# hanyujin02/trajectory_planner

Hardware: AMD Instinct MI355X
Metric: B-spline trajs/s (32 ctrl pts, 256^3 grid, 50 iters) @1 GPU; % HBM roofline (higher is better)
Workload: dtype f64

## Files before the change

trajectory_planner_amd/csrc/vigo_solver.hip:

```cpp
#include <stdlib.h>

#include <type_traits>
#include <utility>

#include "vigo_exact_div.hpp"
#include "vigo_internal.hpp"
#include "vigo_linesearch.hpp"
#include "vigo_solver_plan.hpp"

#ifndef VIGO_AXIS_TS_MARK
#define VIGO_AXIS_TS_MARK 1
#endif
#ifndef VIGO_AXIS_CONV_FILTER
#define VIGO_AXIS_CONV_FILTER 1
#endif
#ifndef VIGO_AXIS_PAIR_EVAL
#define VIGO_AXIS_PAIR_EVAL 1
#endif
#ifndef VIGO_AXIS_PAIR_UPDATE
#define VIGO_AXIS_PAIR_UPDATE 1
#endif
#ifndef VIGO_AXIS_LS_FIRST_TESTS
#define VIGO_AXIS_LS_FIRST_TESTS 0
#endif
#ifndef VIGO_AXIS_LS_FIRST_SETUP
#define VIGO_AXIS_LS_FIRST_SETUP 2
#endif

namespace vigo {
namespace {


__device__ __forceinline__ int dpp_prev_i32(int v) {
    return __builtin_amdgcn_mov_dpp(v, 0x138, 0xF, 0xF, false);
}
__device__ __forceinline__ int dpp_next_i32(int v) {
    return __builtin_amdgcn_mov_dpp(v, 0x130, 0xF, 0xF, false);
}
__device__ __forceinline__ double from_prev(double v) {
    return __hiloint2double(dpp_prev_i32(__double2hiint(v)), dpp_prev_i32(__double2loint(v)));
}
__device__ __forceinline__ double from_next(double v) {
    return __hiloint2double(dpp_next_i32(__double2hiint(v)), dpp_next_i32(__double2loint(v)));
}
__device__ __forceinline__ float from_prev(float v) {
    return __int_as_float(dpp_prev_i32(__float_as_int(v)));
}
__device__ __forceinline__ float from_next(float v) {
    return __int_as_float(dpp_next_i32(__float_as_int(v)));
}

template <typename T, int PPL>
__device__ __forceinline__ void seq_next(const T (&a)[PPL], T (&o)[PPL]) {
    const T edge = from_next(a[0]);
#pragma unroll
    for (int q = 0; q + 1 < PPL; ++q) o[q] = a[q + 1];
    o[PPL - 1] = edge;
}
template <typename T, int PPL>
__device__ __forceinline__ void seq_prev(const T (&a)[PPL], T (&o)[PPL]) {
    const T edge = from_prev(a[PPL - 1]);
#pragma unroll
    for (int q = PPL - 1; q > 0; --q) o[q] = a[q - 1];
    o[0] = edge;
}

template <int CTRL>
__device__ __forceinline__ double dpp_f64(double v) {
    const int lo = __builtin_amdgcn_mov_dpp(__double2loint(v), CTRL, 0xF, 0xF, false);
    const int hi = __builtin_amdgcn_mov_dpp(__double2hiint(v), CTRL, 0xF, 0xF, false);
    return __hiloint2double(hi, lo);
}
__device__ __forceinline__ double add_f64_again(double a, double b) {
    double r;
    asm volatile("v_add_f64 %0, %1, %2" : "=v"(r) : "v"(a), "v"(b));
    return r;
}
__device__ __forceinline__ void xor16_parts(double a, double b, double& p0, double& p1) {
    const int alo = __double2loint(a), ahi = __double2hiint(a), blo = __double2loint(b), bhi = __double2hiint(b);
    auto l = __builtin_amdgcn_permlane16_swap(alo, blo, false, false);
    auto h = __builtin_amdgcn_permlane16_swap(ahi, bhi, false, false);
    p0 = __hiloint2double(h[0], l[0]);
    p1 = __hiloint2double(h[1], l[1]);
}
__device__ __forceinline__ double xor32_sum2(double a, double b) {
    const int alo = __double2loint(a), ahi = __double2hiint(a), blo = __double2loint(b), bhi = __double2hiint(b);
    auto l = __builtin_amdgcn_permlane32_swap(alo, blo, false, false);
    auto h = __builtin_amdgcn_permlane32_swap(ahi, bhi, false, false);
    return __hiloint2double(h[0], l[0]) + __hiloint2double(h[1], l[1]);
}
__device__ __forceinline__ void xy_parts(double a, double b, double& x, double& y) {
    const int alo = __double2loint(a), ahi = __double2hiint(a), blo = __double2loint(b), bhi = __double2hiint(b);
    auto l = __builtin_amdgcn_permlane32_swap(alo, blo, false, false);
    auto h = __builtin_amdgcn_permlane32_swap(ahi, bhi, false, false);
    x = __hiloint2double(h[0], l[0]);
    y = __hiloint2double(h[1], l[1]);
}
__device__ __forceinline__ void xy_both(double v, double& x, double& y) { xy_parts(v, v, x, y); }
__device__ __forceinline__ double mul_f64_again(double a, double b) {
    double r;
    asm volatile("v_mul_f64 %0, %1, %2" : "=v"(r) : "v"(a), "v"(b));
    return r;
}
__device__ __forceinline__ double dot_xy(double a, double b) { return xor32_sum2(a * b, mul_f64_again(a, b)); }

template <int GROUP, int K>
__device__ __forceinline__ void group_sum(double (&v)[K]) {
    static_assert(GROUP == 16 || GROUP == 32 || GROUP == 64, "group is a DPP row, half a wave or a wave");
#pragma unroll
    for (int q = 0; q < K; ++q) v[q] += dpp_f64<0xB1>(v[q]);
#pragma unroll
    for (int q = 0; q < K; ++q) v[q] += dpp_f64<0x4E>(v[q]);
#pragma unroll
    for (int q = 0; q < K; ++q) v[q] += dpp_f64<0x141>(v[q]);
    if (GROUP >= 32) {
#pragma unroll
        for (int q = 0; q < K; ++q) {
            const double t = dpp_f64<0x140>(v[q]);
            const double a = v[q] + t;
            const double b = add_f64_again(v[q], t);
            double p0, p1;
            xor16_parts(a, b, p0, p1);
            if (GROUP == 64) v[q] = xor32_sum2(p0 + p1, add_f64_again(p0, p1));
            else v[q] = p0 + p1;
        }
        return;
    }
#pragma unroll
    for (int q = 0; q < K; ++q) v[q] += dpp_f64<0x140>(v[q]);
}
template <int GROUP>
__device__ __forceinline__ double group_sum1(double v) {
    double a[1] = {v};
    group_sum<GROUP, 1>(a);
    return a[0];
}

template <int K>
__device__ __forceinline__ void pair_tree32(double (&v)[K], double (&a)[K], double (&b)[K]) {
#pragma unroll
    for (int q = 0; q < K; ++q) v[q] += dpp_f64<0xB1>(v[q]);
#pragma unroll
    for (int q = 0; q < K; ++q) v[q] += dpp_f64<0x4E>(v[q]);
#pragma unroll
    for (int q = 0; q < K; ++q) v[q] += dpp_f64<0x141>(v[q]);
#pragma unroll
    for (int q = 0; q < K; ++q) {
        const double t = dpp_f64<0x140>(v[q]);
        double p0, p1;
        xor16_parts(v[q] + t, add_f64_again(v[q], t), p0, p1);
        xy_parts(p0 + p1, add_f64_again(p0, p1), a[q], b[q]);
    }
}
__device__ __forceinline__ double pack_xy(double u, double w) {
    const int ulo = __double2loint(u), uhi = __double2hiint(u), wlo = __double2loint(w), whi = __double2hiint(w);
    auto l = __builtin_amdgcn_permlane32_swap(ulo, wlo, false, false);
    auto h = __builtin_amdgcn_permlane32_swap(uhi, whi, false, false);
    return __hiloint2double(h[0], l[0]) + __hiloint2double(h[1], l[1]);
}
__device__ __forceinline__ void ys_yy_axis(double y, double s, double& ys, double& yy) {
    double v[1] = {pack_xy(y * s, y * y) + 0.0}, a[1], b[1];
    pair_tree32<1>(v, a, b);
    ys = a[0];
    yy = b[0];
}

template <int GROUP>
__device__ __forceinline__ void group_minmax(double& mn, double& mx) {
    static_assert(GROUP == 32 || GROUP == 64, "half a wave or a wave");
    auto step = [&](double omn, double omx) { mn = fmin(mn, omn); mx = fmax(mx, omx); };
    step(dpp_f64<0xB1>(mn), dpp_f64<0xB1>(mx));
    step(dpp_f64<0x4E>(mn), dpp_f64<0x4E>(mx));
    step(dpp_f64<0x141>(mn), dpp_f64<0x141>(mx));
    step(dpp_f64<0x140>(mn), dpp_f64<0x140>(mx));
    {
        double a0, a1, b0, b1;
        xor16_parts(mn, mn, a0, a1);
        xor16_parts(mx, mx, b0, b1);
        mn = fmin(a0, a1);
        mx = fmax(b0, b1);
    }
    if (GROUP == 64) {
        const int nlo = __double2loint(mn), nhi = __double2hiint(mn), xlo = __double2loint(mx), xhi = __double2hiint(mx);
        auto l = __builtin_amdgcn_permlane32_swap(nlo, nlo, false, false);
        auto h = __builtin_amdgcn_permlane32_swap(nhi, nhi, false, false);
        mn = fmin(__hiloint2double(h[0], l[0]), __hiloint2double(h[1], l[1]));
        auto l2 = __builtin_amdgcn_permlane32_swap(xlo, xlo, false, false);
        auto h2 = __builtin_amdgcn_permlane32_swap(xhi, xhi, false, false);
        mx = fmax(__hiloint2double(h2[0], l2[0]), __hiloint2double(h2[1], l2[1]));
    }
}

__device__ __forceinline__ double sum3(double a, double b, double c) { return (a + b) + c; }

__device__ __forceinline__ double fmaT(double a, double b, double c) { return __builtin_fma(a, b, c); }
__device__ __forceinline__ float fmaT(float a, float b, float c) { return __builtin_fmaf(a, b, c); }

template <bool FAST, typename T, int D = 3>
__device__ __forceinline__ double dot3(const T (&a)[3], const T (&b)[3]) {
    if (D == 2) {
        if (FAST) return fmaT((double)a[1], (double)b[1], (double)a[0] * (double)b[0]);
        return (double)a[0] * (double)b[0] + (double)a[1] * (double)b[1];
    }
    if (FAST)
        return fmaT((double)a[2], (double)b[2], fmaT((double)a[1], (double)b[1], (double)a[0] * (double)b[0]));
    return sum3((double)a[0] * (double)b[0], (double)a[1] * (double)b[1], (double)a[2] * (double)b[2]);
}
template <bool FAST, typename T, int PPL, int D = 3>
__device__ __forceinline__ double dot_lane(const T (&a)[PPL][3], const T (&b)[PPL][3]) {
    if constexpr (D == 1) {
        static_assert(!FAST && PPL == 1, "the axis-per-lane layout is reference order, one point per lane pair");
        return dot_xy((double)a[0][0], (double)b[0][0]);
    } else {
        double s = dot3<FAST, T, D>(a[0], b[0]);
#pragma unroll
        for (int q = 1; q < PPL; ++q) s += dot3<FAST, T, D>(a[q], b[q]);
        return s;
    }
}

template <bool FAST>
struct YSv {
    double v, r;
};
template <>
struct YSv<true> {
    double v;
};
__device__ __forceinline__ bool exp_in_safe_range(double a) {
    const unsigned e = ((unsigned)__double2hiint(a) >> 20) & 0x7ffu;
    return (e - 523u) < 1000u;
}
__device__ __forceinline__ YSv<true> make_ys(double ys, YSv<true>*) { return YSv<true>{1.0 / ys}; }
__device__ __forceinline__ YSv<false> make_ys(double ys, YSv<false>*) {
    return YSv<false>{ys, exp_in_safe_range(ys) ? 1.0 / ys : __builtin_nan("")};
}
template <bool MARK>
__device__ __forceinline__ double over_ys(double a, const YSv<true>& y, double&, double&) { return a * y.v; }
template <bool MARK>
__device__ __forceinline__ double over_ys(double a, const YSv<false>& y, double& amin, double& amax) {
    if (!MARK) return a / y.v;
    const double q = a * y.r;
    const double e = __builtin_fma(-q, y.v, a);
    amin = fmin(amin, fabs(a));
    amax = fmax(amax, fabs(a));
    return __builtin_fma(e, y.r, q);
}

template <bool STEADY, bool MARK>
struct TwoLoopTag {
    static constexpr bool value = STEADY;
};
template <bool FAST, bool STEADY>
constexpr bool two_loop_mark(std::integral_constant<bool, STEADY>) { return STEADY && !FAST; }
template <bool FAST, bool STEADY, bool MARK>
constexpr bool two_loop_mark(TwoLoopTag<STEADY, MARK>) { return MARK; }

template <typename T, int D = 3>
struct alignas(16) HPair {
    T s[D];
    T y[D];
};

template <typename T, int PPL>
struct LaneProblem {
    static constexpr int kGuideRegs = (PPL == 1) ? 2 : 0;
    static constexpr int kGuideDim = kGuideRegs > 0 ? kGuideRegs : 1;
    int N;
    bool level;
    int p0;
    bool has_pt[PPL];
    bool interior[PPL];
    int g_begin[PPL], g_end[PPL];
    const double* gpv;
    const uint8_t* gunk;
    T gq[kGuideDim][6];
    bool gqu[kGuideDim];
    int o_begin, o_end;
    const double* obs;
    const double* obs_tab;
    const double* obs_size;
    int o_tab, o_steps;
    double w[4];
};

__device__ __forceinline__ void hold_in_reg(double& v) { asm volatile("" : "+v"(v)); }
__device__ __forceinline__ void hold_in_reg(int& v) { asm volatile("" : "+s"(v)); }
__device__ __forceinline__ void fresh_reg(double& v) { asm volatile("" : "=v"(v)); }
__device__ __forceinline__ void fresh_reg(int& v) { asm volatile("" : "=s"(v)); }
struct HotConst {
    double dth, da, db, dc, unc_factor;
    double ts_ctrl, ts_inv_sqr;
    double g_epsilon, min_step, max_step, ftol, gtol, xtol;
    int max_iterations, max_linesearch;
    double ts_rcp, ts_lim, g_eps2;
    int conv_ok;
    __device__ __forceinline__ explicit HotConst(const DevConst& K)
        : dth(K.dth), da(K.da), db(K.db), dc(K.dc), unc_factor(K.unc_factor), ts_ctrl(K.ts_ctrl), ts_inv_sqr(K.ts_inv_sqr),
          g_epsilon(K.g_epsilon), min_step(K.min_step), max_step(K.max_step), ftol(K.ftol), gtol(K.gtol), xtol(K.xtol),
          max_iterations(K.max_iterations), max_linesearch(K.max_linesearch) {
        hold_in_reg(dth); hold_in_reg(da); hold_in_reg(db); hold_in_reg(dc); hold_in_reg(unc_factor);
        hold_in_reg(ts_ctrl); hold_in_reg(ts_inv_sqr);
        hold_in_reg(g_epsilon); hold_in_reg(min_step); hold_in_reg(max_step); hold_in_reg(ftol); hold_in_reg(gtol); hold_in_reg(xtol);
        hold_in_reg(max_iterations); hold_in_reg(max_linesearch);
        const ConstDiv cd = make_const_div(ts_ctrl);
        const ConvFilter cf = make_conv_filter(g_epsilon);
        ts_rcp = cd.r; ts_lim = cd.lim2; g_eps2 = cf.eps2;
        conv_ok = __builtin_amdgcn_readfirstlane((int)cf.ok);
        hold_in_reg(ts_rcp); hold_in_reg(ts_lim); hold_in_reg(g_eps2); hold_in_reg(conv_ok);
    }
};
template <bool HOT>
using LoopConst = std::conditional_t<HOT, HotConst, const DevConst&>;

template <typename T, class KC>
__device__ __forceinline__ bool guide_penalty(const KC& K, T dist, bool unk, T& ct, T& k, bool& scale) {
    const T dth = (T)K.dth, da = (T)K.da, db = (T)K.db, dcc = (T)K.dc;
    const T e = dth - dist;
    scale = false;
    if (e <= -dth) {
        const T ne = -e;
        ct = (ne * ne) * ne;
        k = T(3.0) * (ne * ne);
    } else if (e > T(0) && e <= dth) {
        ct = (e * e) * e;
        k = T(-3.0) * (e * e);
        scale = unk;
    } else if (e >= dth) {
        ct = (da * (e * e) + db * e) + dcc;
        k = -((T(2) * da) * e + db);
        scale = unk;
    } else {
        return false;
    }
    return true;
}
template <bool FAST, typename T>
__device__ __forceinline__ void guide_pair_term(const DevConst& K, const T (&c)[3], T px, T py, T pz, T vx,
                                                T vy, T vz, bool unk, double& cd, T (&Gd)[3]) {
    const T uf = (T)K.unc_factor;
    const T dist = FAST ? fmaT(c[2] - pz, vz, fmaT(c[1] - py, vy, (c[0] - px) * vx))
                        : ((c[0] - px) * vx + (c[1] - py) * vy) + (c[2] - pz) * vz;
    T ct, k;
    bool scale;
    if (!guide_penalty<T>(K, dist, unk, ct, k, scale)) return;
    T gx = k * vx, gy = k * vy, gz = k * vz;
    if (scale) { ct *= uf; gx *= uf; gy *= uf; gz *= uf; }
    if (!K.plan_in_z) gz = T(0.0);
    cd += (double)ct;
    Gd[0] += gx; Gd[1] += gy; Gd[2] += gz;
}
template <class KC>
__device__ __forceinline__ void guide_pair_term_axis(const KC& K, double c, double cz, double p, double pz, double v, double vz,
                                                     bool unk, double& cd, double& Gd) {
    const double uf = K.unc_factor;
    const double dist = dot_xy(c - p, v) + (cz - pz) * vz;
    double ct, k;
    bool scale;
    if (!guide_penalty<double>(K, dist, unk, ct, k, scale)) return;
    double gc = k * v;
    if (scale) { ct *= uf; gc *= uf; }
    cd += ct;
    Gd += gc;
}

template <typename T>
__device__ __forceinline__ void obstacle_term(const DevConst& K, const T (&c)[3], T opx, T opy, T ovx, T ovy, T size,
                                              double& co, T (&Go)[3]) {
    const T thr0 = (T)K.thr_dyn, oa = (T)K.oa, ob = (T)K.ob, oc = (T)K.oc;
    for (int n = 0; n <= K.pred_num; n += 2) {
        const T tn = (T)((double)n * K.ts);
        const T px = opx + tn * ovx, py = opy + tn * ovy;
        const T thr = (T(1) - (T)(n / K.pred_num) * T(0.2)) * thr0;
        const T dx = c[0] - px, dy = c[1] - py, dz = T(0.0);
        const T nrm = sqrt((dx * dx + dy * dy) + dz * dz);
        const T e = thr - (nrm - size);
        if (e > T(0)) {
            const bool cubic = e <= thr;
            const T ct = cubic ? (e * e) * e : (oa * (e * e) + ob * e) + oc;
            const T k = cubic ? T(-3.0) * (e * e) : -((T(2) * oa) * e + ob);
            co += (double)ct;
            Go[0] += k * (dx / nrm); Go[1] += k * (dy / nrm);
            if (__builtin_expect(!(nrm > T(0) && nrm < (T)INFINITY), 0)) Go[2] += k * (dz / nrm);
        }
    }
}

template <typename T>
__device__ __forceinline__ void obstacle_term_tab(const DevConst& K, const T (&c)[3], const double* tab, int steps,
                                                  T size, double& co, T (&Go)[3]) {
    const T oa = (T)K.oa, ob = (T)K.ob, oc = (T)K.oc;
    for (int s = 0; s < steps; ++s) {
        const T px = (T)tab[3 * s + 0], py = (T)tab[3 * s + 1], thr = (T)tab[3 * s + 2];
        const T dx = c[0] - px, dy = c[1] - py, dz = T(0.0);
        const T nrm = sqrt((dx * dx + dy * dy) + dz * dz);
        const T e = thr - (nrm - size);
        if (e > T(0)) {
            const bool cubic = e <= thr;
            const T ct = cubic ? (e * e) * e : (oa * (e * e) + ob * e) + oc;
            const T k = cubic ? T(-3.0) * (e * e) : -((T(2) * oa) * e + ob);
            co += (double)ct;
            Go[0] += k * (dx / nrm); Go[1] += k * (dy / nrm);
            if (__builtin_expect(!(nrm > T(0) && nrm < (T)INFINITY), 0)) Go[2] += k * (dz / nrm);
        }
    }
}

__device__ __forceinline__ bool axis_converged(const HotConst& K, double G, double X) {
    const int f = conv_filter(G, X, ConvFilter{K.g_eps2, K.conv_ok != 0});
    if (__builtin_expect(!__any(f < 0), 1)) return f != 0;
    double xnorm = sqrt(X);
    const double gnorm = sqrt(G);
    if (xnorm < 1.0) xnorm = 1.0;
    return gnorm / xnorm <= K.g_epsilon;
}

template <typename T, int PPL, bool FAST, class KC>
__device__ __forceinline__ void stencil_axis(const KC& K, const T (&C)[PPL], bool no_terms, double (&jj)[PPL],
                                             double (&vv)[PPL], double (&aa)[PPL], T (&Gs)[PPL], T (&Gf)[PPL]) {
    const T ts = (T)K.ts_ctrl, tis = (T)K.ts_inv_sqr;
    auto excess = [](T v) -> T { return v > T(1.0) ? v - T(1.0) : (v < T(-1.0) ? v + T(1.0) : T(0.0)); };
    T P1[PPL], P2[PPL], P3[PPL];
    seq_next<T, PPL>(C, P1);
    seq_next<T, PPL>(P1, P2);
    seq_next<T, PPL>(P2, P3);
    T gt0[PPL], gv[PPL], ga[PPL];
#pragma unroll
    for (int q = 0; q < PPL; ++q) {
        T J0 = FAST ? fmaT(T(3), P1[q], fmaT(T(-3), P2[q], P3[q])) - C[q]
                    : ((P3[q] - 3 * P2[q]) + 3 * P1[q]) - C[q];
        if (no_terms) J0 = T(0);
        gt0[q] = T(2.0) * J0;
        jj[q] = (double)(J0 * J0);
        constexpr bool kMark = VIGO_AXIS_TS_MARK && std::is_same_v<KC, HotConst> && std::is_same_v<T, double>;
        T evP, gq = T(0);
        if constexpr (kMark) {
            const ConstDiv cd{K.ts_ctrl, K.ts_rcp, K.ts_lim, K.ts_lim};
            T a = P1[q] - C[q];
            if (__builtin_expect(__any(!cd.usable2(a)), 0)) {
                hold_in_reg(a);
                evP = excess(a / ts);
                if (no_terms) evP = T(0);
                gq = (T(2) * evP) / ts;
            } else {
                evP = excess(cd.quotient(a));
                if (no_terms) evP = T(0);
                gq = cd.quotient(T(2) * evP);
            }
        } else {
            evP = excess((P1[q] - C[q]) / ts);
        }
        T eaP = excess((FAST ? fmaT(T(-2), P1[q], P2[q]) + C[q]
                             : (P2[q] - 2 * P1[q]) + C[q]) * tis);
        if (no_terms) { evP = T(0); eaP = T(0); }
        if constexpr (!kMark) gq = (T(2) * evP) / ts;
        gv[q] = gq * tis;
        ga[q] = (T(2) * eaP) * tis;
        vv[q] = (double)((evP * evP) * tis);
        aa[q] = (double)(eaP * eaP);
    }
    T gt1[PPL], gt2[PPL], gt3[PPL], gvM[PPL], gaM1[PPL], gaM2[PPL];
    seq_prev<T, PPL>(gt0, gt1);
    seq_prev<T, PPL>(gt1, gt2);
    seq_prev<T, PPL>(gt2, gt3);
    seq_prev<T, PPL>(gv, gvM);
    seq_prev<T, PPL>(ga, gaM1);
    seq_prev<T, PPL>(gaM1, gaM2);
#pragma unroll
    for (int q = 0; q < PPL; ++q) {
        T acc = gt3[q];
        if (FAST) {
            acc = fmaT(T(-3.0), gt2[q], acc);
            acc = fmaT(T(3.0), gt1[q], acc);
        } else {
            acc += T(-3.0) * gt2[q];
            acc += T(3.0) * gt1[q];
        }
        acc += -gt0[q];
        Gs[q] = acc;
        T fcc = gvM[q];
        fcc += -gv[q];
        fcc += gaM2[q];
        fcc += -(T(2) * gaM1[q]);
        fcc += ga[q];
        Gf[q] = fcc;
    }
}

template <typename T, int GROUP, int PPL, bool FAST, bool OBS = true, int D = 3>
__device__ __forceinline__ double eval_cost_grad(const DevConst& K, const LaneProblem<T, PPL>& Q,
                                                 const T (&c)[PPL][3], const T (&d)[PPL][3], T (&g)[PPL][3],
                                                 double (&sums)[7]) {
    using LP = LaneProblem<T, PPL>;
    const int N = Q.N;
    T Gd[PPL][3], Gs[PPL][3], Gf[PPL][3], Go[PPL][3];
    double pt_s[PPL], pt_f[PPL], pt_d[PPL], pt_o[PPL];
#pragma unroll
    for (int q = 0; q < PPL; ++q) {
        pt_s[q] = pt_f[q] = pt_d[q] = pt_o[q] = 0.0;
#pragma unroll
        for (int a = 0; a < 3; ++a) Gd[q][a] = Go[q][a] = T(0);
    }

    {
        double jj[PPL][3], vv[PPL][3], aa[PPL][3];
#pragma unroll
        for (int a = 0; a < 3; ++a) {
            if (a >= D) {
#pragma unroll
                for (int q = 0; q < PPL; ++q) { jj[q][a] = vv[q][a] = aa[q][a] = 0.0; Gs[q][a] = Gf[q][a] = T(0); }
                continue;
            }
            T C[PPL], GsA[PPL], GfA[PPL];
            double jjA[PPL], vvA[PPL], aaA[PPL];
#pragma unroll
            for (int q = 0; q < PPL; ++q) C[q] = c[q][a];
            stencil_axis<T, PPL, FAST>(K, C, a == 2 && Q.level, jjA, vvA, aaA, GsA, GfA);
#pragma unroll
            for (int q = 0; q < PPL; ++q) { jj[q][a] = jjA[q]; vv[q][a] = vvA[q]; aa[q][a] = aaA[q]; Gs[q][a] = GsA[q]; Gf[q][a] = GfA[q]; }
        }
#pragma unroll
        for (int q = 0; q < PPL; ++q) {
            const int p = Q.p0 + q;
            if (Q.has_pt[q] && p <= N - 4) pt_s[q] = sum3(jj[q][0], jj[q][1], jj[q][2]);
            double cf = 0.0;
            if (Q.has_pt[q] && p <= N - 2) cf = (vv[q][0] + vv[q][1]) + vv[q][2];
            if (Q.has_pt[q] && p <= N - 3) { cf += aa[q][0]; cf += aa[q][1]; cf += aa[q][2]; }
            pt_f[q] = cf;
        }
    }

#pragma unroll
    for (int q = 0; q < PPL; ++q) {
        if (Q.interior[q]) {
            double cd = 0.0;
            const int cnt = Q.g_end[q] - Q.g_begin[q];
#pragma unroll
            for (int j = 0; j < LP::kGuideRegs; ++j) {
                if (j < cnt)
                    guide_pair_term<FAST, T>(K, c[q], Q.gq[j][0], Q.gq[j][1], Q.gq[j][2], Q.gq[j][3], Q.gq[j][4], Q.gq[j][5],
                                       Q.gqu[j], cd, Gd[q]);
            }
            for (int j = Q.g_begin[q] + LP::kGuideRegs; j < Q.g_end[q]; ++j) {
                const double* pv = Q.gpv + 6 * (size_t)j;
                guide_pair_term<FAST, T>(K, c[q], (T)pv[0], (T)pv[1], (T)pv[2], (T)pv[3], (T)pv[4], (T)pv[5],
                                   Q.gunk ? (Q.gunk[j] != 0) : false, cd, Gd[q]);
            }
            if (K.plan_in_z) {
                const T hth = (T)K.hth, ha = (T)K.ha, hb = (T)K.hb, hc = (T)K.hc;
                const T hmin = c[q][2] - (T)K.min_h, hmax = c[q][2] - (T)K.max_h;
                if (hmin < T(0)) {
                    const T e = hth - hmin;
                    cd += (double)((ha * (e * e) + hb * e) + hc);
                    Gd[q][0] += -((T(2) * ha) * e + hb) * T(-1.0);
                } else if (hmin >= T(0) && hmax < hth) {
                    const T e = hth - hmin;
                    cd += (double)((e * e) * e);
                    Gd[q][0] += T(-3.0) * (e * e) * T(-1.0);
                }
                if (hmax > T(0)) {
                    const T e = hth + hmax;
                    cd += (double)((ha * (e * e) + hb * e) + hc);
                    Gd[q][0] += -((T(2) * ha) * e + hb) * T(1.0);
                } else if (hmax <= T(0) && hmax >= -hth) {
                    const T e = hth + hmax;
                    cd += (double)((e * e) * e);
                    Gd[q][0] += T(-3.0) * (e * e) * T(1.0);
                }
            }
            pt_d[q] = cd;
        }
    }

    if (OBS && Q.o_end > Q.o_begin) {
#pragma unroll
        for (int q = 0; q < PPL; ++q) {
            if (!Q.interior[q]) continue;
            double co = 0.0;
            for (int j = 0; j < Q.o_tab; ++j)
                obstacle_term_tab<T>(K, c[q], Q.obs_tab + 3 * j * Q.o_steps, Q.o_steps, (T)Q.obs_size[j], co, Go[q]);
            for (int j = Q.o_begin + Q.o_tab; j < Q.o_end; ++j) {
                const double* o = Q.obs + 9 * (size_t)j;
                const T hx = (T)o[6] / 2, hy = (T)o[7] / 2;
                obstacle_term<T>(K, c[q], (T)o[0], (T)o[1], (T)o[3], (T)o[4], sqrt(hx * hx + hy * hy), co, Go[q]);
            }
            pt_o[q] = co;
        }
    }

    const T w0 = (T)Q.w[0], w1 = (T)Q.w[1], w2 = (T)Q.w[2], w3 = (T)Q.w[3];
    double part[7];
#pragma unroll
    for (int q = 0; q < PPL; ++q) {
#pragma unroll
        for (int a = 0; a < 3; ++a)
            g[q][a] = (!Q.interior[q] || a >= D || (a == 2 && Q.level)) ? T(0)
                      : (FAST ? fmaT(w3, Go[q][a], fmaT(w2, Gf[q][a], fmaT(w1, Gs[q][a], w0 * Gd[q][a])))
                              : ((w0 * Gd[q][a] + w1 * Gs[q][a]) + w2 * Gf[q][a]) + w3 * Go[q][a]);
        const double v4 = dot3<FAST, T, D>(g[q], d[q]);
        const double v5 = Q.interior[q] ? dot3<FAST, T>(c[q], c[q]) : 0.0;
        const double v6 = dot3<FAST, T, D>(g[q], g[q]);
        if (q == 0) {
            part[0] = pt_d[0]; part[1] = pt_s[0]; part[2] = pt_f[0]; part[3] = pt_o[0];
            part[4] = v4; part[5] = v5; part[6] = v6;
        } else {
            part[0] += pt_d[q]; part[1] += pt_s[q]; part[2] += pt_f[q]; part[3] += pt_o[q];
            part[4] += v4; part[5] += v5; part[6] += v6;
        }
    }
    if (OBS) {
        group_sum<GROUP, 7>(part);
    } else {
        double p6[6] = {part[0], part[1], part[2], part[4], part[5], part[6]};
        group_sum<GROUP, 6>(p6);
        part[0] = p6[0]; part[1] = p6[1]; part[2] = p6[2]; part[3] = 0.0; part[4] = p6[3]; part[5] = p6[4]; part[6] = p6[5];
    }
#pragma unroll
    for (int q = 0; q < 7; ++q) sums[q] = part[q];
    return ((Q.w[0] * part[0] + Q.w[1] * part[1]) + Q.w[2] * part[2]) + Q.w[3] * part[3];
}

template <class KC>
__device__ __forceinline__ double eval_cost_grad_axis(const KC& K, const LaneProblem<double, 1>& Q, int axis,
                                                      const double (&c)[1][3], const double (&d)[1][3], double (&g)[1][3],
                                                      double (&sums)[7]) {
    using LP = LaneProblem<double, 1>;
    const int N = Q.N, p = Q.p0;
    const double C[1] = {c[0][0]};
    const double cz = c[0][2];
    double jj[1], vv[1], aa[1], Gs[1], Gf[1];
    stencil_axis<double, 1, false>(K, C, false, jj, vv, aa, Gs, Gf);
    double pt_s = 0.0, pt_f = 0.0, pt_d = 0.0;
    double pt_sf = 0.0;
    if constexpr (VIGO_AXIS_PAIR_EVAL) {
        double a0, a1;
        xy_both(aa[0], a0, a1);
        const double t = pack_xy(jj[0], vv[0]) + 0.0;
        if (Q.has_pt[0] && p <= (axis ? N - 2 : N - 4)) pt_sf = t;
        if (axis && Q.has_pt[0] && p <= N - 3) { pt_sf += a0; pt_sf += a1; pt_sf += 0.0; }
    } else {
        double j0, j1, v0, v1, a0, a1;
        xy_both(jj[0], j0, j1);
        xy_both(vv[0], v0, v1);
        xy_both(aa[0], a0, a1);
        if (Q.has_pt[0] && p <= N - 4) pt_s = sum3(j0, j1, 0.0);
        if (Q.has_pt[0] && p <= N - 2) pt_f = (v0 + v1) + 0.0;
        if (Q.has_pt[0] && p <= N - 3) { pt_f += a0; pt_f += a1; pt_f += 0.0; }
    }

    double Gd = 0.0;
    if (Q.interior[0]) {
        double cd = 0.0;
        const int cnt = Q.g_end[0] - Q.g_begin[0];
#pragma unroll
        for (int j = 0; j < LP::kGuideRegs; ++j) {
            if (j < cnt) guide_pair_term_axis(K, C[0], cz, Q.gq[j][0], Q.gq[j][2], Q.gq[j][3], Q.gq[j][5], Q.gqu[j], cd, Gd);
        }
        for (int j = Q.g_begin[0] + LP::kGuideRegs; j < Q.g_end[0]; ++j) {
            const double* pv = Q.gpv + 6 * (size_t)j;
            guide_pair_term_axis(K, C[0], cz, pv[axis], pv[2], pv[3 + axis], pv[5], Q.gunk ? (Q.gunk[j] != 0) : false, cd, Gd);
        }
        pt_d = cd;
    }

    const double w0 = Q.w[0], w1 = Q.w[1], w2 = Q.w[2], w3 = Q.w[3];
    const double Go = 0.0;
    g[0][0] = !Q.interior[0] ? 0.0 : ((w0 * Gd + w1 * Gs[0]) + w2 * Gf[0]) + w3 * Go;
    g[0][1] = g[0][2] = 0.0;
    if constexpr (VIGO_AXIS_PAIR_EVAL) {
        const double xx = dot_xy(C[0], C[0]) + cz * cz;
        double v3[3], lo[3], hi[3];
        v3[0] = axis ? (Q.interior[0] ? xx : 0.0) : pt_d;
        v3[1] = pt_sf;
        v3[2] = pack_xy(g[0][0] * d[0][0], g[0][0] * g[0][0]);
        pair_tree32<3>(v3, lo, hi);
        sums[0] = lo[0]; sums[1] = lo[1]; sums[2] = hi[1]; sums[3] = 0.0; sums[4] = lo[2]; sums[5] = hi[0]; sums[6] = hi[2];
    } else {
        double p6[6];
        p6[0] = pt_d; p6[1] = pt_s; p6[2] = pt_f;
        p6[3] = dot_xy(g[0][0], d[0][0]);
        const double xx = dot_xy(C[0], C[0]) + cz * cz;
        p6[4] = Q.interior[0] ? xx : 0.0;
        p6[5] = dot_xy(g[0][0], g[0][0]);
        group_sum<32, 6>(p6);
        sums[0] = p6[0]; sums[1] = p6[1]; sums[2] = p6[2]; sums[3] = 0.0; sums[4] = p6[3]; sums[5] = p6[4]; sums[6] = p6[5];
    }
    return ((Q.w[0] * sums[0] + Q.w[1] * sums[1]) + Q.w[2] * sums[2]) + Q.w[3] * sums[3];
}

__device__ __forceinline__ void axis_guides(LaneProblem<double, 1>& Q, int axis) {
#pragma unroll
    for (int j = 0; j < LaneProblem<double, 1>::kGuideDim; ++j) {
        Q.gq[j][0] = axis ? Q.gq[j][1] : Q.gq[j][0];
        Q.gq[j][3] = axis ? Q.gq[j][4] : Q.gq[j][3];
    }
}

template <bool MIXED> using SolveArgsOf = std::conditional_t<MIXED, MixedSolveArgs, SolveArgs>;
template <typename T, int GROUP, int PPL, bool MIXED = false>
__device__ __forceinline__ bool load_problem(const SolveArgsOf<MIXED>& A, const DevConst& K, int b, int lane_in_group,
                                             LaneProblem<T, PPL>& Q) {
    using LP = LaneProblem<T, PPL>;
    int N = A.N;
    bool valid = true;
    if constexpr (MIXED) {
        static_assert(PPL == 1, "mixed counts: one control point per lane (Ns <= 64)");
        const int n = A.n_pts[b];
        valid = n >= 7 && n <= A.N && shape_for(n).group == GROUP;
        N = valid ? n : 0;
    }
    Q.N = N;
    Q.level = false;
    Q.p0 = lane_in_group * PPL;
    Q.gpv = A.guide_pv;
    Q.gunk = A.guide_unk;
#pragma unroll
    for (int q = 0; q < PPL; ++q) {
        const int p = Q.p0 + q;
        Q.has_pt[q] = p < N;
        Q.interior[q] = (p >= 3) && (p <= N - 4);
        Q.g_begin[q] = Q.g_end[q] = 0;
        if (Q.interior[q] && A.guide_off && A.guide_pv) {
            Q.g_begin[q] = A.guide_off[(size_t)b * (MIXED ? A.N : N) + p];
            Q.g_end[q] = A.guide_off[(size_t)b * (MIXED ? A.N : N) + p + 1];
        }
    }
#pragma unroll
    for (int j = 0; j < LP::kGuideDim; ++j) {
        Q.gqu[j] = false;
#pragma unroll
        for (int q = 0; q < 6; ++q) Q.gq[j][q] = T(0);
        if (j < LP::kGuideRegs && Q.g_begin[0] + j < Q.g_end[0]) {
            const double* pv = A.guide_pv + 6 * (size_t)(Q.g_begin[0] + j);
#pragma unroll
            for (int q = 0; q < 6; ++q) Q.gq[j][q] = (T)pv[q];
            Q.gqu[j] = A.guide_unk ? (A.guide_unk[Q.g_begin[0] + j] != 0) : false;
        }
    }
    Q.obs = A.obs;
    Q.obs_tab = Q.obs_size = nullptr;
    Q.o_tab = Q.o_steps = 0;
    if (!A.obs) {
        Q.o_begin = Q.o_end = 0;
    } else if (A.obs_off) {
        Q.o_begin = A.obs_off[b];
        Q.o_end = A.obs_off[b + 1];
    } else {
        Q.o_begin = 0;
        Q.o_end = A.obs ? A.n_obs_shared : 0;
    }
    if (A.weights) {
#pragma unroll
        for (int q = 0; q < 4; ++q) Q.w[q] = A.weights[4 * (size_t)b + q];
    } else {
#pragma unroll
        for (int q = 0; q < 4; ++q) Q.w[q] = K.w[q];
    }
    return valid;
}

template <typename T, int PPL>
__device__ __forceinline__ void load_points(const SolveArgs& A, int b, const LaneProblem<T, PPL>& Q, T (&x)[PPL][3]) {
#pragma unroll
    for (int q = 0; q < PPL; ++q) {
        x[q][0] = x[q][1] = x[q][2] = T(0);
        if (Q.has_pt[q]) {
            const double* src = A.ctrl + ((size_t)b * A.N + Q.p0 + q) * 3;
            x[q][0] = (T)src[0]; x[q][1] = (T)src[1]; x[q][2] = (T)src[2];
        }
    }
}

template <typename T, int GROUP, int PPL>
__device__ __forceinline__ void set_level(const DevConst& K, LaneProblem<T, PPL>& Q, const T (&x)[PPL][3]) {
    double mn = INFINITY, mx = -INFINITY;
#pragma unroll
    for (int q = 0; q < PPL; ++q) {
        if (Q.has_pt[q]) { mn = fmin(mn, (double)x[q][2]); mx = fmax(mx, (double)x[q][2]); }
    }
    group_minmax<GROUP>(mn, mx);
    Q.level = !K.plan_in_z && !K.strict_z && (mx - mn) <= 0x1p-40 * fmax(1.0, fmax(fabs(mn), fabs(mx)));
}

template <typename T, int PPL>
__device__ __forceinline__ void store_points(const SolveArgs& A, int b, const LaneProblem<T, PPL>& Q, const T (&x)[PPL][3]) {
#pragma unroll
    for (int q = 0; q < PPL; ++q) {
        if (Q.has_pt[q]) {
            double* dst = A.ctrl + ((size_t)b * A.N + Q.p0 + q) * 3;
            dst[0] = (double)x[q][0]; dst[1] = (double)x[q][1]; dst[2] = (double)x[q][2];
        }
    }
}

__device__ __forceinline__ void store_point_axis(const SolveArgs& A, int b, const LaneProblem<double, 1>& Q, int axis, double v, double z) {
    if (!Q.has_pt[0]) return;
    double* dst = A.ctrl + ((size_t)b * A.N + Q.p0) * 3;
    dst[axis] = v;
    if (axis == 0) dst[2] = z;
}

template <typename T, int GROUP, int PPL, bool FAST, bool MIXED = false>
__global__ void __launch_bounds__(kWave) k_cost_grad(SolveArgsOf<MIXED> A, const DevConst* __restrict__ Kp) {
    const DevConst& K = *Kp;
    constexpr int TPB = kWave / GROUP;
    const int lane = threadIdx.x;
    const int b = blockIdx.x * TPB + lane / GROUP;
    if (b >= A.B) return;
    LaneProblem<T, PPL> Q;
    if (!load_problem<T, GROUP, PPL, MIXED>(A, K, b, lane % GROUP, Q)) {
        if (lane % GROUP == 0 && A.out_cost) A.out_cost[b] = __builtin_nan("");
        return;
    }
    T c[PPL][3], g[PPL][3], zero[PPL][3];
    load_points<T, PPL>(A, b, Q, c);
    set_level<T, GROUP, PPL>(K, Q, c);
#pragma unroll
    for (int q = 0; q < PPL; ++q) zero[q][0] = zero[q][1] = zero[q][2] = T(0);
    double sums[7];
    const double f = eval_cost_grad<T, GROUP, PPL, FAST>(K, Q, c, zero, g, sums);
#pragma unroll
    for (int q = 0; q < PPL; ++q) {
        if (Q.interior[q] && A.out_grad) {
            double* dst = A.out_grad + ((size_t)b * (A.N - 6) + (Q.p0 + q - 3)) * 3;
            dst[0] = (double)g[q][0]; dst[1] = (double)g[q][1]; dst[2] = (double)g[q][2];
        }
    }
    if (lane % GROUP == 0) {
        if (A.out_cost) A.out_cost[b] = f;
        if (A.out_terms) {
#pragma unroll
            for (int q = 0; q < 4; ++q) A.out_terms[4 * (size_t)b + q] = sums[q];
        }
    }
}

#ifndef VIGO_PROFILE_SECTIONS
#define VIGO_PROFILE_SECTIONS 0
#endif
#if VIGO_PROFILE_SECTIONS
#define VIGO_TICK(acc)                                                   \
    do {                                                                 \
        __builtin_amdgcn_sched_barrier(0);                               \
        const long long now_ = (long long)__builtin_readcyclecounter();  \
        __builtin_amdgcn_sched_barrier(0);                               \
        acc += (double)(now_ - tick_);                                   \
        tick_ = now_;                                                    \
    } while (0)
#else
#define VIGO_TICK(acc) do { } while (0)
#endif

template <typename T, int GROUP, int PPL, bool FAST, int WPS = 1, bool OBS = true, int D = 3, int RH = (PPL == 1 ? 1 : 0), bool MIXED = false>
__global__ void __launch_bounds__(kWave, WPS) k_optimize(SolveArgsOf<MIXED> A, const DevConst* __restrict__ Kp) {
    static_assert(!MIXED || (D == 3 && OBS && PPL == 1), "mixed counts: the general kernel, one point per lane");
    static_assert(PPL == 1 ? (RH >= 1 && RH <= 6) : RH == 0, "register-held history only with one point per lane");
    constexpr bool AXIS = D == 1;
    static_assert(!AXIS || (std::is_same<T, double>::value && GROUP == 32 && PPL == 1 && !FAST && !OBS),
                  "the axis-per-lane layout: fp64 reference order, N <= 32, no obstacles");
    const DevConst& K = *Kp;
    constexpr int TPB = AXIS ? 1 : kWave / GROUP;
    constexpr int COLS = kWave / GROUP;
    extern __shared__ __align__(16) unsigned char lds_raw[];
    const int N = A.N, NI = N - 6;
    const int ROW = COLS * NI;
    const int ROWP = ROW + 1;
    using YS = YSv<FAST>;
    constexpr int kYsSlotBytes = (TPB * (int)sizeof(YS) + 15) & ~15;
    const int slotB = ROWP * (int)sizeof(HPair<T, D>) + kYsSlotBytes;
    const int m = K.mem_size;
    const LoopConst<AXIS> KL(K);
    constexpr bool REG1 = (PPL == 1);
    const int ms = REG1 ? (m > RH + 1 ? m - (RH + 1) : 0) : m;
    HPair<T, D>* hist = reinterpret_cast<HPair<T, D>*>(lds_raw);
    double* ys_tab = reinterpret_cast<double*>(lds_raw + (size_t)ms * slotB);

    const int lane = threadIdx.x;
    const int grp = lane / GROUP;
    const int tg = AXIS ? 0 : grp;
    int b = blockIdx.x * TPB + tg;
    if (A.active_idx) {
        if (b >= *A.active_count) return;
        b = A.active_idx[b];
    } else if (b >= A.B) {
        return;
    }

    LaneProblem<T, PPL> Q;
    const bool valid_n = load_problem<T, GROUP, PPL, MIXED>(A, K, b, lane % GROUP, Q);
    T x[PPL][3];
    load_points<T, PPL>(A, b, Q, x);
    set_level<T, GROUP, PPL>(K, Q, x);
    if constexpr (AXIS) {
        if (!Q.level) return;
        x[0][0] = grp ? x[0][1] : x[0][0];
        axis_guides(Q, grp);
    } else {
        const bool wave_level = __all(Q.level);
        if (D == 2 && !wave_level) return;
        if (D == 3 && A.level_waves_elsewhere && wave_level) return;
    }
    const bool solved_elsewhere = D == 3 && A.level_waves_elsewhere == 2 && Q.level;
#if VIGO_PROFILE_SECTIONS
    long long tick_ = (long long)__builtin_readcyclecounter();
    double t_eval = 0, t_ls = 0, t_upd = 0, t_two = 0, t_tail = 0, t_pre = 0, t_trial = 0, t_cal = 0;
#endif
    HPair<T, D>* hl[PPL];
#pragma unroll
    for (int q = 0; q < PPL; ++q) {
        const int p = Q.p0 + q;
        hl[q] = Q.interior[q] ? hist + (grp * NI + (p - 3)) : hist + ROW;
    }
    for (int slot = lane; slot < ms; slot += kWave) {
        HPair<T, D> zero;
#pragma unroll
        for (int a = 0; a < D; ++a) zero.s[a] = zero.y[a] = T(0);
        *reinterpret_cast<HPair<T, D>*>(lds_raw + (size_t)slot * slotB + (size_t)ROW * sizeof(HPair<T, D>)) = zero;
    }
    __syncthreads();
    if (solved_elsewhere) return;
    if (MIXED && !valid_n) {
        if (lane % GROUP == 0 && A.out_status) A.out_status[(size_t)b * (A.status_stride ? A.status_stride : 1)] = LBERR_INVALID_N;
        return;
    }
    YS* ys_l = reinterpret_cast<YS*>(lds_raw + (size_t)ROWP * sizeof(HPair<T, D>)) + tg;
    double* al_l = ys_tab + tg;
    auto hist_at = [&](int q, int slot) -> HPair<T, D>& {
        return *reinterpret_cast<HPair<T, D>*>(reinterpret_cast<char*>(hl[q]) + (size_t)slot * slotB);
    };
    auto ys_at = [&](int slot) -> YS& { return *reinterpret_cast<YS*>(reinterpret_cast<char*>(ys_l) + (size_t)slot * slotB); };
    if (!OBS) { Q.obs = nullptr; Q.o_begin = Q.o_end = 0; }
    if (OBS && A.obs) {
        constexpr int kEnt = kObsTabEntries<GROUP>;
        double* tab = ys_tab + (size_t)m * TPB + (size_t)grp * kObsTabDoubles<GROUP>;
        const int cnt = Q.o_end - Q.o_begin;
        const int steps = K.pred_num / 2 + 1;
        int fit = kEnt / steps;
        if (fit > kObsTabObs) fit = kObsTabObs;
        Q.o_tab = cnt < fit ? cnt : fit;
        Q.o_steps = steps;
        Q.obs_tab = tab;
        Q.obs_size = tab + 3 * kEnt;
        for (int e = lane % GROUP; e < Q.o_tab * steps; e += GROUP) {
            const int j = e / steps, n = 2 * (e - j * steps);
            const double* o = A.obs + 9 * (size_t)(Q.o_begin + j);
            const T tn = (T)((double)n * K.ts);
            tab[3 * e + 0] = (double)((T)o[0] + tn * (T)o[3]);
            tab[3 * e + 1] = (double)((T)o[1] + tn * (T)o[4]);
            tab[3 * e + 2] = (double)((T(1) - (T)(n / K.pred_num) * T(0.2)) * (T)K.thr_dyn);
        }
        for (int j = lane % GROUP; j < Q.o_tab; j += GROUP) {
            const double* o = A.obs + 9 * (size_t)(Q.o_begin + j);
            const T hx = (T)o[6] / 2, hy = (T)o[7] / 2;
            tab[3 * kEnt + j] = (double)(T)sqrt(hx * hx + hy * hy);
        }
        __syncthreads();
    }

    T g[PPL][3], xp[PPL][3], gp[PPL][3], d[PPL][3];
#pragma unroll
    for (int q = 0; q < PPL; ++q)
#pragma unroll
        for (int a = 0; a < 3; ++a) g[q][a] = xp[q][a] = gp[q][a] = d[q][a] = T(0);
    constexpr int kRH = RH > 0 ? RH : 1;
    T sR[kRH][PPL][3], yR[kRH][PPL][3];
    YS ysR[kRH]{};
#pragma unroll
    for (int q = 0; q < PPL; ++q)
#pragma unroll
        for (int a = 0; a < 3; ++a)
#pragma unroll
            for (int j = 0; j < kRH; ++j) sR[j][q][a] = yR[j][q][a] = T(0);
    T dz = T(-0.0);
    double sums[7];
    int evals = 0;
    int ret = LBERR_UNKNOWN;
    int k = 0, end = 0, last = 0;
    double fx = 0.0, step = 0.0;
    bool first = true;

    for (;;) {
        int ls = 0;
        if constexpr (AXIS && (VIGO_AXIS_LS_FIRST_TESTS || VIGO_AXIS_LS_FIRST_SETUP)) {
            constexpr bool kTests = VIGO_AXIS_LS_FIRST_TESTS, kDefer = VIGO_AXIS_LS_FIRST_SETUP == 1;
            const LsParams P{KL.min_step, KL.max_step, KL.ftol, KL.gtol, KL.xtol, KL.max_linesearch};
            LsState S;
            fresh_reg(S.dginit); fresh_reg(S.finit); fresh_reg(S.dgtest); fresh_reg(S.width); fresh_reg(S.prev_width);
            fresh_reg(S.xt); fresh_reg(S.xf); fresh_reg(S.xd); fresh_reg(S.yt); fresh_reg(S.yf); fresh_reg(S.yd);
            fresh_reg(S.stmin); fresh_reg(S.stmax);
            fresh_reg(S.count); fresh_reg(S.brackt); fresh_reg(S.stage1); fresh_reg(S.uinfo);
            double step0 = step;
            auto move_x = [&]() {
                x[0][0] = xp[0][0] + step * d[0][0];
                x[0][2] = xp[0][2] + step * (Q.interior[0] ? dz : 0.0);
            };
            bool run = true;
            if (!first) {
                xp[0][0] = x[0][0]; gp[0][0] = g[0][0];
                xp[0][2] = x[0][2];
                ls = kDefer ? ls_first_begin(P, S, step, fx, sums[4]) : ls_begin(P, S, step, fx, sums[4]);
                run = ls == 0;
                if (run) {
                    if constexpr (kDefer) ls_first_setup(P, step);
                    else ls_setup(P, S, step);
                    move_x();
                }
            }
            while (run) {
                VIGO_TICK(t_pre);
                fx = eval_cost_grad_axis(KL, Q, grp, x, d, g, sums);
                VIGO_TICK(t_eval);
                ++evals;
                if (first) break;

                const double dg = sums[4];
                const double ftest1 = ls_ftest1(S, step);
                ++S.count;
                if ((kTests || kDefer) && S.count == 1) {
                    if constexpr (kTests) {
                        const int code = ls_first_exit_code(P, S, step, fx, dg, ftest1);
                        if (__any(code != 0)) { ls = code; break; }
                    }
                    if constexpr (kDefer) {
                        hold_in_reg(step0);
                        ls_first_reject(P, S, step0);
                        hold_in_reg(S.xt); hold_in_reg(S.xf); hold_in_reg(S.xd); hold_in_reg(S.yt); hold_in_reg(S.yf); hold_in_reg(S.yd);
                        hold_in_reg(S.width); hold_in_reg(S.prev_width); hold_in_reg(S.stmin); hold_in_reg(S.stmax);
                        hold_in_reg(S.brackt); hold_in_reg(S.stage1); hold_in_reg(S.uinfo);
                    }
                }
                if (!kTests || S.count != 1) {
                    const int code = ls_exit_code(P, S, step, fx, dg, ftest1);
                    if (code != 0) { ls = code; break; }
                }
                VIGO_TICK(t_ls);
                ls_update(P, S, step, fx, dg, ftest1);
                VIGO_TICK(t_trial);
                ls_setup(P, S, step);
                move_x();
            }
        } else {
            int count = 0, brackt = 0, stage1 = 1, uinfo = 0;
            double dginit = 0.0, finit = 0.0, dgtest = 0.0, width = 0.0, prev_width = 0.0;
            double xt = 0., xf = 0., xd = 0., yt = 0., yf = 0., yd = 0.;
            const double stpmin = KL.min_step, stpmax = KL.max_step;
            bool run = true;
            if (!first) {
#pragma unroll
                for (int q = 0; q < PPL; ++q)
#pragma unroll
                    for (int a = 0; a < D; ++a) { xp[q][a] = x[q][a]; gp[q][a] = g[q][a]; }
                if constexpr (AXIS) xp[0][2] = x[0][2];
                dginit = sums[4];
                if (step <= 0.) { ls = LBERR_INVALIDPARAMETERS; run = false; }
                else if (0 < dginit) { ls = LBERR_INCREASEGRADIENT; run = false; }
                finit = fx;
                dgtest = KL.ftol * dginit;
                width = stpmax - stpmin;
                prev_width = 2.0 * width;
                xt = yt = 0.;
                xf = yf = finit;
                xd = yd = dginit;
            }
            while (run) {
                double stmin = 0., stmax = 0.;
                if (!first) {
                    if (brackt) {
                        stmin = xt <= yt ? xt : yt;
                        stmax = xt >= yt ? xt : yt;
                    } else {
                        stmin = xt;
                        stmax = step + 4.0 * (step - xt);
                    }
                    if (step < stpmin) step = stpmin;
                    if (stpmax < step) step = stpmax;
                    if ((brackt && ((step <= stmin || stmax <= step) || KL.max_linesearch <= count + 1 || uinfo != 0)) ||
                        (brackt && (stmax - stmin <= KL.xtol * stmax))) {
                        step = xt;
                    }
#pragma unroll
                    for (int q = 0; q < PPL; ++q)
#pragma unroll
                        for (int a = 0; a < D; ++a)
                            x[q][a] = FAST ? fmaT((T)step, d[q][a], xp[q][a]) : xp[q][a] + (T)step * d[q][a];
                    if constexpr (AXIS) x[0][2] = xp[0][2] + (T)step * (Q.interior[0] ? dz : T(0));
                }

                VIGO_TICK(t_pre);
                if constexpr (AXIS) fx = eval_cost_grad_axis(KL, Q, grp, x, d, g, sums);
                else fx = eval_cost_grad<T, GROUP, PPL, FAST, OBS, D>(KL, Q, x, d, g, sums);
                VIGO_TICK(t_eval);
                ++evals;
                if (first) break;

                const double dg = sums[4];
                const double ftest1 = finit + step * dgtest;
                ++count;

                {
                    int code = 0;
                    if (fx <= ftest1 && fabs(dg) <= KL.gtol * (-dginit)) code = count;
                    if (KL.max_linesearch <= count) code = LBERR_MAXIMUMLINESEARCH;
                    if (brackt && (stmax - stmin) <= KL.xtol * stmax) code = LBERR_WIDTHTOOSMALL;
                    if (step == stpmin && (ftest1 < fx || dgtest <= dg)) code = LBERR_MINIMUMSTEP;
                    if (step == stpmax && fx <= ftest1 && dg <= dgtest) code = LBERR_MAXIMUMSTEP;
                    if (brackt && ((step <= stmin || stmax <= step) || uinfo != 0)) code = LBERR_ROUNDING_ERROR;
                    if (code != 0) { ls = code; break; }
                }

                const double cmin = KL.ftol <= KL.gtol ? KL.ftol : KL.gtol;
                if (stage1 && fx <= ftest1 && cmin * dginit <= dg) stage1 = 0;

                const bool mod = stage1 && ftest1 < fx && fx <= xf;
                double axf = mod ? xf - xt * dgtest : xf, axd = mod ? xd - dgtest : xd;
                double ayf = mod ? yf - yt * dgtest : yf, ayd = mod ? yd - dgtest : yd;
                const double atf = mod ? fx - step * dgtest : fx, atd = mod ? dg - dgtest : dg;
                VIGO_TICK(t_ls);
                uinfo = trial_interval(xt, axf, axd, yt, ayf, ayd, step, atf, atd, stmin, stmax, brackt);
                VIGO_TICK(t_trial);
                xf = mod ? axf + xt * dgtest : axf;
                yf = mod ? ayf + yt * dgtest : ayf;
                xd = mod ? axd + dgtest : axd;
                yd = mod ? ayd + dgtest : ayd;

                if (brackt) {
                    if (0.66 * prev_width <= fabs(yt - xt)) step = xt + 0.5 * (yt - xt);
                    prev_width = width;
                    width = fabs(yt - xt);
                }
            }
        }

        VIGO_TICK(t_ls);
        double xnorm = sqrt(sums[5]), gnorm = sqrt(sums[6]);
        if (first) {
            first = false;
#pragma unroll
            for (int q = 0; q < PPL; ++q)
#pragma unroll
                for (int a = 0; a < D; ++a) d[q][a] = -g[q][a];
            if constexpr (AXIS && VIGO_AXIS_CONV_FILTER) {
                if (axis_converged(KL, sums[6], sums[5])) { ret = LB_ALREADY_MINIMIZED; break; }
            } else {
                if (xnorm < 1.0) xnorm = 1.0;
                if (gnorm / xnorm <= KL.g_epsilon) { ret = LB_ALREADY_MINIMIZED; break; }
            }
            step = 1.0 / sqrt(sums[6]);
            sums[4] = -sums[6];
            k = 1;
            end = 0;
            continue;
        }

        if (ls < 0) {
            if constexpr (AXIS) store_point_axis(A, b, Q, grp, Q.interior[0] ? x[0][0] : xp[0][0], Q.interior[0] ? x[0][2] : xp[0][2]);
            else store_points<T, PPL>(A, b, Q, x);
#pragma unroll
            for (int q = 0; q < PPL; ++q)
#pragma unroll
                for (int a = 0; a < D; ++a) { x[q][a] = xp[q][a]; g[q][a] = gp[q][a]; }
            if constexpr (AXIS) x[0][2] = xp[0][2];
            ret = ls;
            break;
        }

        if constexpr (AXIS && VIGO_AXIS_CONV_FILTER) {
            if (axis_converged(KL, sums[6], sums[5])) { ret = LB_CONVERGENCE; break; }
        } else {
            if (xnorm < 1.0) xnorm = 1.0;
            if (gnorm / xnorm <= KL.g_epsilon) { ret = LB_CONVERGENCE; break; }
        }
        if (KL.max_iterations != 0 && KL.max_iterations < k + 1) { ret = LBERR_MAXIMUMITERATION; break; }

        T sv[PPL][3], yv[PPL][3];
#pragma unroll
        for (int q = 0; q < PPL; ++q) {
#pragma unroll
            for (int a = 0; a < D; ++a) { sv[q][a] = x[q][a] - xp[q][a]; yv[q][a] = g[q][a] - gp[q][a]; }
            if (!REG1 && Q.interior[q]) {
                HPair<T, D> hp;
#pragma unroll
                for (int a = 0; a < D; ++a) { hp.s[a] = sv[q][a]; hp.y[a] = yv[q][a]; }
                hist_at(q, end) = hp;
            }
        }
        double ysyy[2];
        if constexpr (AXIS && VIGO_AXIS_PAIR_UPDATE) {
            ys_yy_axis(yv[0][0], sv[0][0], ysyy[0], ysyy[1]);
        } else {
            ysyy[0] = dot_lane<FAST, T, PPL, D>(yv, sv);
            ysyy[1] = dot_lane<FAST, T, PPL, D>(yv, yv);
            if (D <= 2) ysyy[0] += 0.0;
            group_sum<GROUP, 2>(ysyy);
        }
        const double ys = ysyy[0], yy = ysyy[1];
        const YS ys_div = make_ys(ys, static_cast<YS*>(nullptr));
        if (!REG1) ys_at(end) = ys_div;
        const bool haveR = REG1 && k >= RH + 1;

        const int bound = (m <= k) ? m : k;
        const int newest = REG1 ? last : end;
        if (!REG1) end = (end + 1 == m) ? 0 : end + 1;
        ++k;
#pragma unroll
        for (int q = 0; q < PPL; ++q)
#pragma unroll
            for (int a = 0; a < D; ++a) d[q][a] = -g[q][a];

        constexpr int kWin = 2;
        T Ps[kWin][PPL][3], Py[kWin][PPL][3];
        YS Pys[kWin];
        auto fetch = [&](int age, T (&s_)[PPL][3], T (&y_)[PPL][3], YS& ys_) {
            if (REG1 && age == 0) {
#pragma unroll
                for (int q = 0; q < PPL; ++q)
#pragma unroll
                    for (int a = 0; a < D; ++a) { s_[q][a] = sv[q][a]; y_[q][a] = yv[q][a]; }
                ys_ = ys_div;
                return;
            }
            if (REG1 && age >= 1 && age <= RH) {
                const int j = (age - 1 < kRH && age >= 1) ? age - 1 : 0;
#pragma unroll
                for (int q = 0; q < PPL; ++q)
#pragma unroll
                    for (int a = 0; a < D; ++a) { s_[q][a] = sR[j][q][a]; y_[q][a] = yR[j][q][a]; }
                ys_ = ysR[j];
                return;
            }
            int slot = REG1 ? newest - (age - (RH + 1)) : newest - age;
            if (slot < 0) slot += ms;
#pragma unroll
            for (int q = 0; q < PPL; ++q) {
                const HPair<T, D> h = hist_at(q, slot);
#pragma unroll
                for (int a = 0; a < D; ++a) { s_[q][a] = h.s[a]; y_[q][a] = h.y[a]; }
            }
            ys_ = ys_at(slot);
        };
        auto two_loop = [&](auto steady_tag) -> bool {
            constexpr bool STEADY = decltype(steady_tag)::value;
            constexpr bool MARK = two_loop_mark<FAST>(decltype(steady_tag){});
            double amin = 1.0, amax = 1.0;
            const int bnd = STEADY ? kMaxMem : __builtin_amdgcn_readfirstlane(bound);
            constexpr bool REGAL = STEADY || AXIS;
            double al_reg[REGAL ? kMaxMem : 1];
            constexpr int kRing = kMaxMem - (RH + 1);
            constexpr int kFirstRing = RH + 1;
            const int stepB = slotB;
            const int lastU = STEADY ? __builtin_amdgcn_readfirstlane(last) : 0;
            int curB = lastU * stepB;
            auto ring_fetch = [&](T (&s_)[PPL][3], T (&y_)[PPL][3], YS& ys_) {
#pragma unroll
                for (int q = 0; q < PPL; ++q) {
                    const HPair<T, D> h = *reinterpret_cast<const HPair<T, D>*>(reinterpret_cast<const char*>(hl[q]) + curB);
#pragma unroll
                    for (int a = 0; a < D; ++a) { s_[q][a] = h.s[a]; y_[q][a] = h.y[a]; }
                }
                ys_ = *reinterpret_cast<const YS*>(reinterpret_cast<const char*>(ys_l) + curB);
            };
            auto ring_older = [&]() {
                curB -= stepB;
                if (curB < 0) curB += kRing * stepB;
            };
            auto ring_newer = [&]() {
                curB += stepB;
                if (curB >= kRing * stepB) curB -= kRing * stepB;
            };
            auto ring_fetch_age = [&](int age, bool newer_next, T (&s_)[PPL][3], T (&y_)[PPL][3], YS& ys_) {
                ring_fetch(s_, y_, ys_);
                if (newer_next) ring_newer(); else ring_older();
            };
#pragma unroll
            for (int q = 0; q < PPL; ++q)
#pragma unroll
                for (int a = 0; a < D; ++a) { Ps[0][q][a] = sv[q][a]; Py[0][q][a] = yv[q][a]; }
            Pys[0] = ys_div;
#pragma unroll
            for (int age = 1; age < kWin; ++age)
                if (age < bnd) {
                    if (STEADY && age >= kFirstRing) ring_fetch_age(age, false, Ps[age], Py[age], Pys[age]);
                    else fetch(age, Ps[age], Py[age], Pys[age]);
                }
#pragma unroll
            for (int age = 0; age < kMaxMem; ++age) {
                if (age < bnd) {
                    const int w = age % kWin;
                    double al = group_sum1<GROUP>(dot_lane<FAST, T, PPL, D>(Ps[w], d));
                    al = over_ys<MARK>(al, Pys[w], amin, amax);
                    if (REGAL) al_reg[REGAL ? age : 0] = al;
                    else al_l[age * TPB] = al;
                    {
                        const T na = (T)(-al);
#pragma unroll
                        for (int q = 0; q < PPL; ++q)
#pragma unroll
                            for (int a = 0; a < D; ++a) d[q][a] = FAST ? fmaT(na, Py[w][q][a], d[q][a]) : d[q][a] + na * Py[w][q][a];
                    }
                    if (age + kWin < kMaxMem && age + kWin < bnd) {
                        if (STEADY && age + kWin >= kFirstRing) ring_fetch_age(age + kWin, false, Ps[w], Py[w], Pys[w]);
                        else fetch(age + kWin, Ps[w], Py[w], Pys[w]);
                    }
                }
            }
            if (STEADY) {
#pragma unroll
                for (int i = 0; i < kWin + 1; ++i) ring_newer();
                asm volatile("" ::: "memory");
            }
            {
                const T sc = (T)(ys / yy);
#pragma unroll
                for (int q = 0; q < PPL; ++q)
#pragma unroll
                    for (int a = 0; a < D; ++a) d[q][a] *= sc;
            }
#pragma unroll
            for (int age = kMaxMem - 1; age >= 0; --age) {
                if (age < bnd) {
                    const int w = age % kWin;
                    double beta = group_sum1<GROUP>(dot_lane<FAST, T, PPL, D>(Py[w], d));
                    beta = over_ys<MARK>(beta, Pys[w], amin, amax);
                    const double cod = (REGAL ? al_reg[REGAL ? age : 0] : al_l[age * TPB]) - beta;
                    {
                        const T co = (T)cod;
#pragma unroll
                        for (int q = 0; q < PPL; ++q)
#pragma unroll
                            for (int a = 0; a < D; ++a) d[q][a] = FAST ? fmaT(co, Ps[w][q][a], d[q][a]) : d[q][a] + co * Ps[w][q][a];
                    }
                    if (age - kWin >= 0) {
                        if (STEADY && age - kWin >= kFirstRing) ring_fetch_age(age - kWin, true, Ps[w], Py[w], Pys[w]);
                        else fetch(age - kWin, Ps[w], Py[w], Pys[w]);
                    }
                }
            }
            if (!MARK) return false;
            bool bad = !(amin >= 0x1p-500) || !(amax <= 0x1p500);
#pragma unroll
            for (int q = 0; q < PPL; ++q)
#pragma unroll
                for (int a = 0; a < D; ++a) bad |= !(d[q][a] == d[q][a]);
            return bad;
        };
        VIGO_TICK(t_upd);
        if constexpr (AXIS) {
            bool bad;
            if (bound == kMaxMem && !__any(last != __builtin_amdgcn_readfirstlane(last))) bad = two_loop(TwoLoopTag<true, true>{});
            else bad = two_loop(TwoLoopTag<false, true>{});
            if (__any(bad)) {
                asm volatile("" ::: "memory");
                d[0][0] = -g[0][0];
                two_loop(TwoLoopTag<false, false>{});
            }
        } else if (PPL == 1 && bound == kMaxMem && !__any(last != __builtin_amdgcn_readfirstlane(last))) {
            if (__any(two_loop(std::true_type{}))) {
                asm volatile("" ::: "memory");
#pragma unroll
                for (int q = 0; q < PPL; ++q)
#pragma unroll
                    for (int a = 0; a < D; ++a) d[q][a] = -g[q][a];
                two_loop(std::false_type{});
            }
        } else {
            two_loop(std::false_type{});
        }
        if constexpr (AXIS)
            dz = __hiloint2double(__builtin_amdgcn_readfirstlane(__double2hiint(d[0][0])),
                                  __builtin_amdgcn_readfirstlane(__double2loint(d[0][0])));
#pragma unroll
        for (int q = 0; q < PPL; ++q)
#pragma unroll
            for (int a = 0; a < D; ++a) d[q][a] = Q.interior[q] ? d[q][a] : T(0);
        VIGO_TICK(t_two);
        if (REG1) {
            if (haveR && ms > 0) {
#pragma unroll
                for (int q = 0; q < PPL; ++q) {
                    if (Q.interior[q]) {
                        HPair<T, D> hp;
#pragma unroll
                        for (int a = 0; a < D; ++a) { hp.s[a] = sR[kRH - 1][q][a]; hp.y[a] = yR[kRH - 1][q][a]; }
                        hist_at(q, end) = hp;
                    }
                }
                ys_at(end) = ysR[kRH - 1];
                last = end;
                end = (end + 1 == ms) ? 0 : end + 1;
            }
#pragma unroll
            for (int j = kRH - 1; j > 0; --j) {
#pragma unroll
                for (int q = 0; q < PPL; ++q)
#pragma unroll
                    for (int a = 0; a < D; ++a) { sR[j][q][a] = sR[j - 1][q][a]; yR[j][q][a] = yR[j - 1][q][a]; }
                ysR[j] = ysR[j - 1];
            }
#pragma unroll
            for (int q = 0; q < PPL; ++q)
#pragma unroll
                for (int a = 0; a < D; ++a) { sR[0][q][a] = sv[q][a]; yR[0][q][a] = yv[q][a]; }
            ysR[0] = ys_div;
        }
        sums[4] = group_sum1<GROUP>(dot_lane<FAST, T, PPL, D>(g, d));
        step = 1.0;
        VIGO_TICK(t_tail);
        VIGO_TICK(t_cal);
    }

    if (ret >= 0 || ret == LBERR_MAXIMUMITERATION) {
        if constexpr (AXIS) store_point_axis(A, b, Q, grp, x[0][0], x[0][2]);
        else store_points<T, PPL>(A, b, Q, x);
    }
#pragma unroll
    for (int q = 0; q < PPL; ++q) {
        if (Q.interior[q] && A.out_x) {
            double* dst = A.out_x + ((size_t)b * NI + (Q.p0 + q - 3)) * 3;
            if constexpr (AXIS) {
                dst[grp] = (double)x[q][0];
                if (grp == 0) dst[2] = (double)x[q][2];
            } else {
                dst[0] = (double)x[q][0]; dst[1] = (double)x[q][1]; dst[2] = (double)x[q][2];
            }
        }
    }
#if VIGO_PROFILE_SECTIONS
    if (lane % GROUP == 0 && A.out_x) {
        double* o = A.out_x + (size_t)b * NI * 3;
        o[0] = t_eval; o[1] = t_ls; o[2] = t_upd; o[3] = t_two; o[4] = t_tail; o[5] = (double)k; o[6] = (double)evals;
        o[7] = t_pre; o[8] = t_trial; o[9] = t_cal;
    }
#endif
    if (lane % (kWave / TPB) == 0) {
        if (A.out_status) A.out_status[(size_t)b * (A.status_stride ? A.status_stride : 1)] = ret;
        if (A.out_fx) A.out_fx[b] = fx;
        if (A.out_iters) A.out_iters[b] = k;
        if (A.out_evals) A.out_evals[b] = evals;
    }
}

}

#ifndef VIGO_SOLVER_PART
#define VIGO_SOLVER_PART 0
#endif

using SolveKernel = void (*)(SolveArgs, const DevConst*);
using MixedSolveKernel = void (*)(MixedSolveArgs, const DevConst*);

#if VIGO_SOLVER_PART == 0
DevConst make_dev_const(const vigo_params_t& P) {
    DevConst K{};
    K.dth = P.dthresh;
    K.da = 3.0 * P.dthresh;
    K.db = -3.0 * pow(P.dthresh, 2);
    K.dc = pow(P.dthresh, 3);
    K.unc_factor = P.uncertain_factor;
    K.hth = 0.2;
    K.ha = 3.0 * K.hth;
    K.hb = -3 * pow(K.hth, 2);
    K.hc = pow(K.hth, 3);
    K.min_h = P.min_height;
    K.max_h = P.max_height;
    K.ts_ctrl = P.ts_ctrl;
    K.ts_inv_sqr = 1 / pow(P.ts_ctrl, 2);
    K.ts = P.ts;
    K.thr_dyn = P.dist_thresh_dynamic;
    K.oa = 3.0 * P.dist_thresh_dynamic;
    K.ob = -3 * pow(P.dist_thresh_dynamic, 2);
    K.oc = pow(P.dist_thresh_dynamic, 3);
    K.pred_num = (int)(P.pred_horizon / P.ts);
    K.plan_in_z = P.plan_in_z;
    K.strict_z = P.strict_z != 0;
    K.w[0] = P.w_distance; K.w[1] = P.w_smoothness; K.w[2] = P.w_feasibility; K.w[3] = P.w_dynamic;
    K.mem_size = P.mem_size;
    K.max_iterations = P.max_iterations;
    K.max_linesearch = P.max_linesearch;
    K.g_epsilon = P.g_epsilon;
    K.min_step = P.min_step;
    K.max_step = P.max_step;
    K.ftol = P.f_dec_coeff;
    K.gtol = P.s_curv_coeff;
    K.xtol = P.xtol;
    return K;
}

int launch_cost_grad(hipStream_t s, const SolveArgs& a, const DevConst&, const DevConst* kd, int precision) {
    if (a.B <= 0) return hipSuccess;
    static constexpr SolveKernel kernels[3][4] = {
        {&k_cost_grad<float, 32, 1, false>, &k_cost_grad<float, 64, 1, false>, &k_cost_grad<float, 64, 2, false>, &k_cost_grad<float, 64, 4, false>},
        {&k_cost_grad<double, 32, 1, true>, &k_cost_grad<double, 64, 1, true>, &k_cost_grad<double, 64, 2, true>, &k_cost_grad<double, 64, 4, true>},
        {&k_cost_grad<double, 32, 1, false>, &k_cost_grad<double, 64, 1, false>, &k_cost_grad<double, 64, 2, false>, &k_cost_grad<double, 64, 4, false>}};
    const Shape sh = shape_for(a.N);
    const int tpb = kWave / sh.group;
    const SolveKernel kernel = kernels[precision == VIGO_PREC_F32 ? 0 : (precision == VIGO_PREC_F64_FAST ? 1 : 2)]
                                      [sh.ppl == 1 ? sh.group / 64 : sh.ppl / 2 + 1];
    hipLaunchKernelGGL(kernel, dim3((a.B + tpb - 1) / tpb), dim3(kWave), 0, s, a, kd);
    return (int)hipGetLastError();
}
#endif


template <int I>
static constexpr SolveKernel optimize_kernel_of() {
    constexpr OptimizeKey k = kOptimizeKeys[I];
    if constexpr (VIGO_SOLVER_PART <= 1 && k.obs == (VIGO_SOLVER_PART == 1)) {
        using T = std::conditional_t<k.precision == VIGO_PREC_F32, float, double>;
        constexpr bool FAST = k.precision == VIGO_PREC_F64_FAST;
        static_assert(sizeof(T) == elem_bytes_of(k.precision) && sizeof(HPair<T, k.d>) == hpair_bytes(sizeof(T), k.d) &&
                          sizeof(YSv<FAST>) == ysv_bytes(FAST), "optimize_lds_bytes computes these sizes by arithmetic");
        return &k_optimize<T, k.group, k.ppl, FAST, k.wps, k.obs, k.d, k.rh>;
    }
    return nullptr;
}
template <class Rows> struct OptimizeKernelTable;
template <int... I> struct OptimizeKernelTable<std::integer_sequence<int, I...>> { static constexpr SolveKernel row[] = {optimize_kernel_of<I>()...}; };
static SolveKernel optimize_kernel(int key) { return OptimizeKernelTable<std::make_integer_sequence<int, kOptimizeKeyCount>>::row[key]; }

#if VIGO_SOLVER_PART == 2
template <int I>
static constexpr MixedSolveKernel optimize_mixed_kernel_of() {
    constexpr OptimizeKey k = kOptimizeMixedKeys[I];
    using T = std::conditional_t<k.precision == VIGO_PREC_F32, float, double>;
    constexpr bool FAST = k.precision == VIGO_PREC_F64_FAST;
    static_assert(sizeof(T) == elem_bytes_of(k.precision) && sizeof(HPair<T, k.d>) == hpair_bytes(sizeof(T), k.d) &&
                      sizeof(YSv<FAST>) == ysv_bytes(FAST), "optimize_lds_bytes computes these sizes by arithmetic");
    return &k_optimize<T, k.group, k.ppl, FAST, k.wps, k.obs, k.d, k.rh, true>;
}
template <class Rows> struct OptimizeMixedKernelTable;
template <int... I> struct OptimizeMixedKernelTable<std::integer_sequence<int, I...>> { static constexpr MixedSolveKernel row[] = {optimize_mixed_kernel_of<I>()...}; };
MixedSolveKernel optimize_mixed_kernel(int key) { return OptimizeMixedKernelTable<std::make_integer_sequence<int, kOptimizeMixedKeyCount>>::row[key]; }
MixedSolveKernel cost_grad_mixed_kernel(int precision, int group) {
    static constexpr MixedSolveKernel kernels[3][2] = {
        {&k_cost_grad<float, 32, 1, false, true>, &k_cost_grad<float, 64, 1, false, true>},
        {&k_cost_grad<double, 32, 1, true, true>, &k_cost_grad<double, 64, 1, true, true>},
        {&k_cost_grad<double, 32, 1, false, true>, &k_cost_grad<double, 64, 1, false, true>}};
    return kernels[precision == VIGO_PREC_F32 ? 0 : (precision == VIGO_PREC_F64_FAST ? 1 : 2)][group / 64];
}
#elif VIGO_SOLVER_PART == 1
SolveKernel optimize_kernel_with_obstacles(int key) { return optimize_kernel(key); }
#else
SolveKernel optimize_kernel_with_obstacles(int key);
MixedSolveKernel optimize_mixed_kernel(int key);
MixedSolveKernel cost_grad_mixed_kernel(int precision, int group);
#ifndef VIGO_EXP_AXIS_SWITCH
#define VIGO_EXP_AXIS_SWITCH 0
#endif
static inline bool axis_dispatch_on() {
#if VIGO_EXP_AXIS_SWITCH
    const char* e = getenv("VIGO_EXP_AXIS");
    return !(e && e[0] == '0');
#else
    return true;
#endif
}

int launch_optimize(hipStream_t s, const SolveArgs& a_in, const DevConst& k, const DevConst* kd, int precision, LaunchState& L) {
    static_assert(kOptimizeKeyCount <= 8 * (int)sizeof(L.lds_attr_set), "one bit per k_optimize instantiation");
    if (a_in.B <= 0) return hipSuccess;
    const OptimizePlan plan = plan_optimize(a_in.N, a_in.B, precision, a_in.obs != nullptr, k.plan_in_z != 0, k.strict_z != 0,
                                            k.mem_size, L.simd_count, axis_dispatch_on());
    if (plan.count < 0) return (int)hipErrorInvalidValue;
    SolveArgs a = a_in;
    for (int i = 0; i < plan.count; ++i) {
        const PlannedLaunch& p = plan.launch[i];
        const SolveKernel kernel = kOptimizeKeys[p.key].obs ? optimize_kernel_with_obstacles(p.key) : optimize_kernel(p.key);
        const uint64_t bit = 1ull << p.key;
        if (p.lds > kLdsStaticLimit && !(L.lds_attr_set & bit)) {
            hipError_t e = hipFuncSetAttribute(reinterpret_cast<const void*>(kernel), hipFuncAttributeMaxDynamicSharedMemorySize, (int)kLdsPerWorkgroup);
            if (e != hipSuccess) return (int)e;
            L.lds_attr_set |= bit;
        }
        a.level_waves_elsewhere = p.level_waves_elsewhere;
        hipLaunchKernelGGL(kernel, dim3(p.grid), dim3(kWave), p.lds, s, a, kd);
        if (hipError_t e = hipGetLastError(); e != hipSuccess) return (int)e;
    }
    return (int)hipSuccess;
}

int launch_cost_grad_mixed(hipStream_t s, const MixedSolveArgs& a, const DevConst* kd, int precision) {
    if (a.B <= 0) return hipSuccess;
    const Shape sh = shape_for(a.N);
    if (sh.ppl != 1 || !a.n_pts) return (int)hipErrorInvalidValue;
    const int tpb = kWave / sh.group;
    hipLaunchKernelGGL(cost_grad_mixed_kernel(precision, sh.group), dim3((a.B + tpb - 1) / tpb), dim3(kWave), 0, s, a, kd);
    return (int)hipGetLastError();
}
int launch_optimize_mixed(hipStream_t s, const MixedSolveArgs& a_in, const DevConst& k, const DevConst* kd, int precision, LaunchState& L) {
    if (a_in.B <= 0) return hipSuccess;
    const OptimizePlan plan = plan_optimize_mixed(a_in.N, a_in.B, precision, a_in.obs != nullptr, k.mem_size, L.simd_count);
    if (plan.count != 1 || !a_in.n_pts) return (int)hipErrorInvalidValue;
    const PlannedLaunch& p = plan.launch[0];
    MixedSolveArgs a = a_in;
    a.level_waves_elsewhere = p.level_waves_elsewhere;
    hipLaunchKernelGGL(optimize_mixed_kernel(p.key), dim3(p.grid), dim3(kWave), p.lds, s, a, kd);
    return (int)hipGetLastError();
}
#endif

}
```

trajectory_planner_amd/csrc/vigo_solver_plan.hpp:

```cpp
#pragma once
#include <stddef.h>

#include "../../include/vigo.h"

namespace vigo {

constexpr int kWave = 64;
constexpr size_t kLdsPerWorkgroup = 160 * 1024;
constexpr size_t kLdsStaticLimit = 64 * 1024;
constexpr int kMaxMem = VIGO_MAX_MEM_SIZE;
constexpr int kObsTabObs = 16;
template <int GROUP> constexpr int kObsTabEntries = GROUP == 32 ? 88 : 33;
template <int GROUP> constexpr int kObsTabDoubles = 3 * kObsTabEntries<GROUP> + kObsTabObs;
constexpr int kLevelRH = 4, kLevelRH64 = 5;
struct Shape { int group, ppl; };
constexpr Shape shape_for(int N) { return N <= 32 ? Shape{32, 1} : Shape{64, N <= 64 ? 1 : (N <= 128 ? 2 : 4)}; }
constexpr int default_rh(int ppl) { return ppl == 1 ? 1 : 0; }
constexpr size_t elem_bytes_of(int precision) { return precision == VIGO_PREC_F32 ? 4 : 8; }
constexpr size_t hpair_bytes(size_t elem_bytes, int D) { return (2 * D * elem_bytes + 15) & ~(size_t)15; }
constexpr size_t ysv_bytes(bool fast) { return fast ? 8 : 16; }

constexpr size_t optimize_lds_bytes(size_t elem_bytes, int group, bool fast, int D, int N, int m, int ppl, bool with_obstacles, int rh) {
    const int TPB = D == 1 ? 1 : kWave / group;
    const int COLS = kWave / group;
    const int ms = ppl == 1 ? (m > rh + 1 ? m - (rh + 1) : 0) : m;
    const size_t slot = ((size_t)COLS * (N - 6) + 1) * hpair_bytes(elem_bytes, D) + (((size_t)TPB * ysv_bytes(fast) + 15) & ~(size_t)15);
    size_t h = (size_t)ms * slot;
    h += (size_t)m * TPB * sizeof(double);
    if (with_obstacles) h += (size_t)TPB * (group == 32 ? kObsTabDoubles<32> : kObsTabDoubles<64>) * sizeof(double);
    return h;
}

constexpr size_t optimize_lds_requirement(int N, int mem_size, int precision) {
    const Shape sh = shape_for(N);
    return optimize_lds_bytes(elem_bytes_of(precision), sh.group, precision == VIGO_PREC_F64_FAST, 3, N, mem_size, sh.ppl, true, default_rh(sh.ppl));
}

struct OptimizeKey { int precision, group, ppl, wps; bool obs; int d, rh; };
constexpr int kF32 = VIGO_PREC_F32, kFast = VIGO_PREC_F64_FAST, kF64 = VIGO_PREC_F64;
constexpr OptimizeKey kOptimizeKeys[] = {
    {kF32, 32, 1, 2, false, 2, 1}, {kF32, 32, 1, 1, false, 2, 1}, {kF32, 32, 1, 2, false, 3, 1}, {kF32, 32, 1, 1, false, 3, 1},
    {kF32, 64, 1, 2, false, 2, 1}, {kF32, 64, 1, 1, false, 2, 1}, {kF32, 64, 1, 2, false, 3, 1}, {kF32, 64, 1, 1, false, 3, 1},
    {kF32, 64, 2, 1, false, 3, 0}, {kF32, 64, 4, 1, false, 3, 0},
    {kFast, 32, 1, 2, false, 2, kLevelRH}, {kFast, 32, 1, 2, false, 2, 1}, {kFast, 32, 1, 1, false, 2, 1}, {kFast, 32, 1, 2, false, 3, 1}, {kFast, 32, 1, 1, false, 3, 1},
    {kFast, 64, 1, 2, false, 2, kLevelRH64}, {kFast, 64, 1, 2, false, 2, 1}, {kFast, 64, 1, 1, false, 2, 1}, {kFast, 64, 1, 2, false, 3, 1}, {kFast, 64, 1, 1, false, 3, 1},
    {kFast, 64, 2, 1, false, 3, 0}, {kFast, 64, 4, 1, false, 3, 0},
    {kF64, 32, 1, 1, false, 1, 1},
    {kF64, 32, 1, 2, false, 2, kLevelRH}, {kF64, 32, 1, 2, false, 2, 1}, {kF64, 32, 1, 1, false, 2, 1}, {kF64, 32, 1, 2, false, 3, 1}, {kF64, 32, 1, 1, false, 3, 1},
    {kF64, 64, 1, 2, false, 2, kLevelRH64}, {kF64, 64, 1, 2, false, 2, 1}, {kF64, 64, 1, 1, false, 2, 1}, {kF64, 64, 1, 2, false, 3, 1}, {kF64, 64, 1, 1, false, 3, 1},
    {kF64, 64, 2, 1, false, 3, 0}, {kF64, 64, 4, 1, false, 3, 0},
    {kF32, 32, 1, 2, true, 3, 1}, {kF32, 32, 1, 1, true, 3, 1}, {kF32, 64, 1, 2, true, 3, 1}, {kF32, 64, 1, 1, true, 3, 1},
    {kF32, 64, 2, 1, true, 3, 0}, {kF32, 64, 4, 1, true, 3, 0},
    {kFast, 32, 1, 2, true, 3, 1}, {kFast, 32, 1, 1, true, 3, 1}, {kFast, 64, 1, 2, true, 3, 1}, {kFast, 64, 1, 1, true, 3, 1},
    {kFast, 64, 2, 1, true, 3, 0}, {kFast, 64, 4, 1, true, 3, 0},
    {kF64, 32, 1, 2, true, 3, 1}, {kF64, 32, 1, 1, true, 3, 1}, {kF64, 64, 1, 2, true, 3, 1}, {kF64, 64, 1, 1, true, 3, 1},
    {kF64, 64, 2, 1, true, 3, 0}, {kF64, 64, 4, 1, true, 3, 0},
};
constexpr int kOptimizeKeyCount = sizeof(kOptimizeKeys) / sizeof(kOptimizeKeys[0]);
constexpr int optimize_key_index(const OptimizeKey& k) {
    for (int i = 0; i < kOptimizeKeyCount; ++i) {
        const OptimizeKey& c = kOptimizeKeys[i];
        if (c.precision == k.precision && c.group == k.group && c.ppl == k.ppl && c.wps == k.wps && c.obs == k.obs && c.d == k.d && c.rh == k.rh) return i;
    }
    return -1;
}

struct PlannedLaunch { int key, grid; size_t lds; int level_waves_elsewhere; };
struct OptimizePlan { int count; PlannedLaunch launch[2]; };

inline OptimizePlan plan_optimize(int N, int B, int precision, bool has_obstacle_list, bool plan_in_z, bool strict_z, int mem_size, int simd_count, bool allow_axis) {
    const Shape sh = shape_for(N);
    const size_t eb = elem_bytes_of(precision);
    const bool fast = precision == VIGO_PREC_F64_FAST, f64 = precision == VIGO_PREC_F64;
    const bool obs = has_obstacle_list || (fast && N > 32 && N <= 64 && simd_count > 0 && B > simd_count && (plan_in_z || strict_z));
    const int grid = (B + kWave / sh.group - 1) / (kWave / sh.group);
    const bool crowded = grid > (simd_count > 0 ? simd_count : (1 << 30));
    auto lds_of = [&](int D, bool table, int rh) { return optimize_lds_bytes(eb, sh.group, fast, D, N, mem_size, sh.ppl, table, rh); };
    auto wps_for = [&](size_t lds) { return sh.ppl == 1 && crowded && lds <= kLdsPerWorkgroup / 8 ? 2 : 1; };
    OptimizePlan p{};
    auto add = [&](int wps, int D, int rh, int g, size_t lds, int lwe) {
        const int key = optimize_key_index(OptimizeKey{precision, sh.group, sh.ppl, wps, obs, D, rh});
        if (key < 0 || p.count < 0) p.count = -1;
        else p.launch[p.count++] = PlannedLaunch{key, g, lds, lwe};
    };
    const size_t lds = lds_of(3, has_obstacle_list, default_rh(sh.ppl));
    if (lds > kLdsPerWorkgroup) return OptimizePlan{-1, {}};
    int lwe = 0;
    if (sh.ppl == 1 && !obs && !plan_in_z && !strict_z) {
        lwe = 1;
        const int rh = sh.group == 32 ? kLevelRH : kLevelRH64;
        const size_t lds2 = lds_of(2, false, 1), lds3 = lds_of(2, false, rh);
        if (f64 && sh.group == 32 && simd_count > 0 && B <= simd_count && allow_axis) {
            add(1, 1, 1, B, lds_of(1, false, 1), lwe);
            lwe = 2;
        } else if (precision != VIGO_PREC_F32 && crowded && lds2 > kLdsPerWorkgroup / 8 && kLdsPerWorkgroup / lds3 > kLdsPerWorkgroup / lds2) {
            add(2, 2, rh, grid, lds3, lwe);
        } else {
            add(wps_for(lds2), 2, 1, grid, lds2, lwe);
        }
    }
    add(wps_for(lds), 3, default_rh(sh.ppl), grid, lds, lwe);
    return p;
}

constexpr int kMixedMaxStride = 64;
constexpr OptimizeKey kOptimizeMixedKeys[] = {
    {kF32, 32, 1, 2, true, 3, 1}, {kF32, 32, 1, 1, true, 3, 1}, {kF32, 64, 1, 2, true, 3, 1}, {kF32, 64, 1, 1, true, 3, 1},
    {kFast, 32, 1, 2, true, 3, 1}, {kFast, 32, 1, 1, true, 3, 1}, {kFast, 64, 1, 2, true, 3, 1}, {kFast, 64, 1, 1, true, 3, 1},
    {kF64, 32, 1, 2, true, 3, 1}, {kF64, 32, 1, 1, true, 3, 1}, {kF64, 64, 1, 2, true, 3, 1}, {kF64, 64, 1, 1, true, 3, 1},
};
constexpr int kOptimizeMixedKeyCount = sizeof(kOptimizeMixedKeys) / sizeof(kOptimizeMixedKeys[0]);
constexpr int optimize_mixed_key_index(int precision, int group, int wps) {
    for (int i = 0; i < kOptimizeMixedKeyCount; ++i) {
        const OptimizeKey& c = kOptimizeMixedKeys[i];
        if (c.precision == precision && c.group == group && c.wps == wps) return i;
    }
    return -1;
}
constexpr bool mixed_count_ok(int n, int Ns) { return n >= 7 && n <= Ns && Ns <= kMixedMaxStride && shape_for(n).group == shape_for(Ns).group; }

inline OptimizePlan plan_optimize_mixed(int Ns, int B, int precision, bool , int mem_size, int simd_count) {
    if (Ns < 7 || Ns > kMixedMaxStride) return OptimizePlan{-1, {}};
    const Shape sh = shape_for(Ns);
    const int grid = (B + kWave / sh.group - 1) / (kWave / sh.group);
    const bool crowded = grid > (simd_count > 0 ? simd_count : (1 << 30));
    const size_t lds = optimize_lds_bytes(elem_bytes_of(precision), sh.group, precision == VIGO_PREC_F64_FAST, 3, Ns, mem_size, 1, true, 1);
    const int key = optimize_mixed_key_index(precision, sh.group, crowded && lds <= kLdsPerWorkgroup / 8 ? 2 : 1);
    if (key < 0 || lds > kLdsStaticLimit) return OptimizePlan{-1, {}};
    return OptimizePlan{1, {PlannedLaunch{key, grid, lds, 0}, {}}};
}

}
```

Measured before the change: 3.897 million.

## Fuse axis-per-lane and general optimize kernels into one launch per trajectory

Moves the optimize kernel body into a shared include and adds a fused kernel. Each block loads its problem once, then branches to the axis-per-lane solver for level trajectories or to a noinline solo general solver otherwise. This replaces the previous two-launch plan (axis kernel, then a general kernel that skipped already-solved waves) and removes one launch plus the redundant problem load. The cost is a larger register footprint from combining both paths, and LDS sized for the larger of the two.

New measurement: 3.956 million, median of 6. 1.5% higher.

```diff
diff --git a/trajectory_planner_amd/csrc/vigo_solver.hip b/trajectory_planner_amd/csrc/vigo_solver.hip
--- a/trajectory_planner_amd/csrc/vigo_solver.hip
+++ b/trajectory_planner_amd/csrc/vigo_solver.hip
@@ -853,589 +853,87 @@
 
 template <typename T, int GROUP, int PPL, bool FAST, int WPS = 1, bool OBS = true, int D = 3, int RH = (PPL == 1 ? 1 : 0), bool MIXED = false>
 __global__ void __launch_bounds__(kWave, WPS) k_optimize(SolveArgsOf<MIXED> A, const DevConst* __restrict__ Kp) {
-    static_assert(!MIXED || (D == 3 && OBS && PPL == 1), "mixed counts: the general kernel, one point per lane");
-    static_assert(PPL == 1 ? (RH >= 1 && RH <= 6) : RH == 0, "register-held history only with one point per lane");
-    constexpr bool AXIS = D == 1;
-    static_assert(!AXIS || (std::is_same<T, double>::value && GROUP == 32 && PPL == 1 && !FAST && !OBS),
-                  "the axis-per-lane layout: fp64 reference order, N <= 32, no obstacles");
+    constexpr bool SOLO = false;
+#define VIGO_OPTIMIZE_ENTRY 1
+#include "vigo_solver_optimize.inc"
+#undef VIGO_OPTIMIZE_ENTRY
+}
+
+template <typename T, int GROUP, int PPL, bool FAST, bool OBS, int D, bool SOLO>
+__device__ __forceinline__ void optimize_loaded(const SolveArgs& A, const DevConst& K, const LoopConst<D == 1>& KL, const int b,
+                                                LaneProblem<T, PPL>& Q, T (&x)[PPL][3]) {
+    constexpr int RH = 1;
+    constexpr bool MIXED = false;
+    const bool valid_n = true;
+#define VIGO_OPTIMIZE_ENTRY 0
+#include "vigo_solver_optimize.inc"
+#undef VIGO_OPTIMIZE_ENTRY
+}
+
+#ifndef VIGO_FUSED_JOIN
+#define VIGO_FUSED_JOIN 0
+#endif
+#if VIGO_FUSED_JOIN == 2
+struct FusedKernArgs { SolveArgs A; const DevConst* Kp; };
+template <class P>
+__device__ __forceinline__ const P& uniform_constant(const void* p) {
+    const unsigned long long u = (unsigned long long)p;
+    const unsigned long long lo = (unsigned)__builtin_amdgcn_readfirstlane((int)(unsigned)u);
+    const unsigned long long hi = (unsigned)__builtin_amdgcn_readfirstlane((int)(unsigned)(u >> 32));
+    typedef const P __attribute__((address_space(4))) * CP;
+    return *(const P*)(CP)((hi << 32) | lo);
+}
+__device__ __noinline__ void optimize_solo(const void* kernargs, const int b_in, const LaneProblem<double, 1>& Q_in, const double (&x_in)[1][3]) {
+    const FusedKernArgs& F = uniform_constant<FusedKernArgs>(kernargs);
+    const DevConst& K = uniform_constant<DevConst>(F.Kp);
+    const int b = __builtin_amdgcn_readfirstlane(b_in);
+    LaneProblem<double, 1> Q = Q_in;
+    double x[1][3] = {{x_in[0][0], x_in[0][1], x_in[0][2]}};
+    optimize_loaded<double, 32, 1, false, false, 3, true>(F.A, K, K, b, Q, x);
+}
+#elif VIGO_FUSED_JOIN == 0
+__device__ __noinline__ void optimize_solo(const SolveArgs& A, const DevConst* Kp, const int b, LaneProblem<double, 1>& Q, double (&x)[1][3]) {
+    optimize_loaded<double, 32, 1, false, false, 3, true>(A, *Kp, *Kp, b, Q, x);
+}
+#endif
+template <int WPS>
+__global__ void __launch_bounds__(kWave, WPS) k_optimize_fused(SolveArgs A, const DevConst* __restrict__ Kp) {
     const DevConst& K = *Kp;
-    constexpr int TPB = AXIS ? 1 : kWave / GROUP;
-    constexpr int COLS = kWave / GROUP;
-    extern __shared__ __align__(16) unsigned char lds_raw[];
-    const int N = A.N, NI = N - 6;
-    const int ROW = COLS * NI;
-    const int ROWP = ROW + 1;
-    using YS = YSv<FAST>;
-    constexpr int kYsSlotBytes = (TPB * (int)sizeof(YS) + 15) & ~15;
-    const int slotB = ROWP * (int)sizeof(HPair<T, D>) + kYsSlotBytes;
-    const int m = K.mem_size;
-    const LoopConst<AXIS> KL(K);
-    constexpr bool REG1 = (PPL == 1);
-    const int ms = REG1 ? (m > RH + 1 ? m - (RH + 1) : 0) : m;
-    HPair<T, D>* hist = reinterpret_cast<HPair<T, D>*>(lds_raw);
-    double* ys_tab = reinterpret_cast<double*>(lds_raw + (size_t)ms * slotB);
-
+    const HotConst KL(K);
     const int lane = threadIdx.x;
-    const int grp = lane / GROUP;
-    const int tg = AXIS ? 0 : grp;
-    int b = blockIdx.x * TPB + tg;
+    const int grp = lane / 32;
+    int b = blockIdx.x;
     if (A.active_idx) {
         if (b >= *A.active_count) return;
         b = A.active_idx[b];
     } else if (b >= A.B) {
         return;
     }
-
-    LaneProblem<T, PPL> Q;
-    const bool valid_n = load_problem<T, GROUP, PPL, MIXED>(A, K, b, lane % GROUP, Q);
-    T x[PPL][3];
-    load_points<T, PPL>(A, b, Q, x);
-    set_level<T, GROUP, PPL>(K, Q, x);
-    if constexpr (AXIS) {
-        if (!Q.level) return;
+    LaneProblem<double, 1> Q;
+    load_problem<double, 32, 1>(A, K, b, lane % 32, Q);
+    double x[1][3];
+    load_points<double, 1>(A, b, Q, x);
+    set_level<double, 32, 1>(K, Q, x);
+    if (__builtin_amdgcn_readfirstlane((int)Q.level)) {
         x[0][0] = grp ? x[0][1] : x[0][0];
         axis_guides(Q, grp);
+        optimize_loaded<double, 32, 1, false, false, 1, false>(A, K, KL, b, Q, x);
     } else {
-        const bool wave_level = __all(Q.level);
-        if (D == 2 && !wave_level) return;
-        if (D == 3 && A.level_waves_elsewhere && wave_level) return;
-    }
-    const bool solved_elsewhere = D == 3 && A.level_waves_elsewhere == 2 && Q.level;
-#if VIGO_PROFILE_SECTIONS
-    long long tick_ = (long long)__builtin_readcyclecounter();
-    double t_eval = 0, t_ls = 0, t_upd = 0, t_two = 0, t_tail = 0, t_pre = 0, t_trial = 0, t_cal = 0;
-#endif
-    HPair<T, D>* hl[PPL];
-#pragma unroll
-    for (int q = 0; q < PPL; ++q) {
-        const int p = Q.p0 + q;
-        hl[q] = Q.interior[q] ? hist + (grp * NI + (p - 3)) : hist + ROW;
-    }
-    for (int slot = lane; slot < ms; slot += kWave) {
-        HPair<T, D> zero;
-#pragma unroll
-        for (int a = 0; a < D; ++a) zero.s[a] = zero.y[a] = T(0);
-        *reinterpret_cast<HPair<T, D>*>(lds_raw + (size_t)slot * slotB + (size_t)ROW * sizeof(HPair<T, D>)) = zero;
-    }
-    __syncthreads();
-    if (solved_elsewhere) return;
-    if (MIXED && !valid_n) {
-        if (lane % GROUP == 0 && A.out_status) A.out_status[(size_t)b * (A.status_stride ? A.status_stride : 1)] = LBERR_INVALID_N;
-        return;
-    }
-    YS* ys_l = reinterpret_cast<YS*>(lds_raw + (size_t)ROWP * sizeof(HPair<T, D>)) + tg;
-    double* al_l = ys_tab + tg;
-    auto hist_at = [&](int q, int slot) -> HPair<T, D>& {
-        return *reinterpret_cast<HPair<T, D>*>(reinterpret_cast<char*>(hl[q]) + (size_t)slot * slotB);
-    };
-    auto ys_at = [&](int slot) -> YS& { return *reinterpret_cast<YS*>(reinterpret_cast<char*>(ys_l) + (size_t)slot * slotB); };
-    if (!OBS) { Q.obs = nullptr; Q.o_begin = Q.o_end = 0; }
-    if (OBS && A.obs) {
-        constexpr int kEnt = kObsTabEntries<GROUP>;
-        double* tab = ys_tab + (size_t)m * TPB + (size_t)grp * kObsTabDoubles<GROUP>;
-        const int cnt = Q.o_end - Q.o_begin;
-        const int steps = K.pred_num / 2 + 1;
-        int fit = kEnt / steps;
-        if (fit > kObsTabObs) fit = kObsTabObs;
-        Q.o_tab = cnt < fit ? cnt : fit;
-        Q.o_steps = steps;
-        Q.obs_tab = tab;
-        Q.obs_size = tab + 3 * kEnt;
-        for (int e = lane % GROUP; e < Q.o_tab * steps; e += GROUP) {
-            const int j = e / steps, n = 2 * (e - j * steps);
-            const double* o = A.obs + 9 * (size_t)(Q.o_begin + j);
-            const T tn = (T)((double)n * K.ts);
-            tab[3 * e + 0] = (double)((T)o[0] + tn * (T)o[3]);
-            tab[3 * e + 1] = (double)((T)o[1] + tn * (T)o[4]);
-            tab[3 * e + 2] = (double)((T(1) - (T)(n / K.pred_num) * T(0.2)) * (T)K.thr_dyn);
-        }
-        for (int j = lane % GROUP; j < Q.o_tab; j += GROUP) {
-            const double* o = A.obs + 9 * (size_t)(Q.o_begin + j);
-            const T hx = (T)o[6] / 2, hy = (T)o[7] / 2;
-            tab[3 * kEnt + j] = (double)(T)sqrt(hx * hx + hy * hy);
-        }
-        __syncthreads();
-    }
-
-    T g[PPL][3], xp[PPL][3], gp[PPL][3], d[PPL][3];
-#pragma unroll
-    for (int q = 0; q < PPL; ++q)
-#pragma unroll
-        for (int a = 0; a < 3; ++a) g[q][a] = xp[q][a] = gp[q][a] = d[q][a] = T(0);
-    constexpr int kRH = RH > 0 ? RH : 1;
-    T sR[kRH][PPL][3], yR[kRH][PPL][3];
-    YS ysR[kRH]{};
-#pragma unroll
-    for (int q = 0; q < PPL; ++q)
-#pragma unroll
-        for (int a = 0; a < 3; ++a)
-#pragma unroll
-            for (int j = 0; j < kRH; ++j) sR[j][q][a] = yR[j][q][a] = T(0);
-    T dz = T(-0.0);
-    double sums[7];
-    int evals = 0;
-    int ret = LBERR_UNKNOWN;
-    int k = 0, end = 0, last = 0;
-    double fx = 0.0, step = 0.0;
-    bool first = true;
-
-    for (;;) {
-        int ls = 0;
-        if constexpr (AXIS && (VIGO_AXIS_LS_FIRST_TESTS || VIGO_AXIS_LS_FIRST_SETUP)) {
-            constexpr bool kTests = VIGO_AXIS_LS_FIRST_TESTS, kDefer = VIGO_AXIS_LS_FIRST_SETUP == 1;
-            const LsParams P{KL.min_step, KL.max_step, KL.ftol, KL.gtol, KL.xtol, KL.max_linesearch};
-            LsState S;
-            fresh_reg(S.dginit); fresh_reg(S.finit); fresh_reg(S.dgtest); fresh_reg(S.width); fresh_reg(S.prev_width);
-            fresh_reg(S.xt); fresh_reg(S.xf); fresh_reg(S.xd); fresh_reg(S.yt); fresh_reg(S.yf); fresh_reg(S.yd);
-            fresh_reg(S.stmin); fresh_reg(S.stmax);
-            fresh_reg(S.count); fresh_reg(S.brackt); fresh_reg(S.stage1); fresh_reg(S.uinfo);
-            double step0 = step;
-            auto move_x = [&]() {
-                x[0][0] = xp[0][0] + step * d[0][0];
-                x[0][2] = xp[0][2] + step * (Q.interior[0] ? dz : 0.0);
-            };
-            bool run = true;
-            if (!first) {
-                xp[0][0] = x[0][0]; gp[0][0] = g[0][0];
-                xp[0][2] = x[0][2];
-                ls = kDefer ? ls_first_begin(P, S, step, fx, sums[4]) : ls_begin(P, S, step, fx, sums[4]);
-                run = ls == 0;
-                if (run) {
-                    if constexpr (kDefer) ls_first_setup(P, step);
-                    else ls_setup(P, S, step);
-                    move_x();
-                }
-            }
-            while (run) {
-                VIGO_TICK(t_pre);
-                fx = eval_cost_grad_axis(KL, Q, grp, x, d, g, sums);
-                VIGO_TICK(t_eval);
-                ++evals;
-                if (first) break;
-
-                const double dg = sums[4];
-                const double ftest1 = ls_ftest1(S, step);
-                ++S.count;
-                if ((kTests || kDefer) && S.count == 1) {
-                    if constexpr (kTests) {
-                        const int code = ls_first_exit_code(P, S, step, fx, dg, ftest1);
-                        if (__any(code != 0)) { ls = code; break; }
-                    }
-                    if constexpr (kDefer) {
-                        hold_in_reg(step0);
-                        ls_first_reject(P, S, step0);
-                        hold_in_reg(S.xt); hold_in_reg(S.xf); hold_in_reg(S.xd); hold_in_reg(S.yt); hold_in_reg(S.yf); hold_in_reg(S.yd);
-                        hold_in_reg(S.width); hold_in_reg(S.prev_width); hold_in_reg(S.stmin); hold_in_reg(S.stmax);
-                        hold_in_reg(S.brackt); hold_in_reg(S.stage1); hold_in_reg(S.uinfo);
-                    }
-                }
-                if (!kTests || S.count != 1) {
-                    const int code = ls_exit_code(P, S, step, fx, dg, ftest1);
-                    if (code != 0) { ls = code; break; }
-                }
-                VIGO_TICK(t_ls);
-                ls_update(P, S, step, fx, dg, ftest1);
-                VIGO_TICK(t_trial);
-                ls_setup(P, S, step);
-                move_x();
-            }
-        } else {
-            int count = 0, brackt = 0, stage1 = 1, uinfo = 0;
-            double dginit = 0.0, finit = 0.0, dgtest = 0.0, width = 0.0, prev_width = 0.0;
-            double xt = 0., xf = 0., xd = 0., yt = 0., yf = 0., yd = 0.;
-            const double stpmin = KL.min_step, stpmax = KL.max_step;
-            bool run = true;
-            if (!first) {
-#pragma unroll
-                for (int q = 0; q < PPL; ++q)
-#pragma unroll
-                    for (int a = 0; a < D; ++a) { xp[q][a] = x[q][a]; gp[q][a] = g[q][a]; }
-                if constexpr (AXIS) xp[0][2] = x[0][2];
-                dginit = sums[4];
-                if (step <= 0.) { ls = LBERR_INVALIDPARAMETERS; run = false; }
-                else if (0 < dginit) { ls = LBERR_INCREASEGRADIENT; run = false; }
-                finit = fx;
-                dgtest = KL.ftol * dginit;
-                width = stpmax - stpmin;
-                prev_width = 2.0 * width;
-                xt = yt = 0.;
-                xf = yf = finit;
-                xd = yd = dginit;
-            }
-            while (run) {
-                double stmin = 0., stmax = 0.;
-                if (!first) {
-                    if (brackt) {
-                        stmin = xt <= yt ? xt : yt;
-                        stmax = xt >= yt ? xt : yt;
-                    } else {
-                        stmin = xt;
-                        stmax = step + 4.0 * (step - xt);
-                    }
-                    if (step < stpmin) step = stpmin;
-                    if (stpmax < step) step = stpmax;
-                    if ((brackt && ((step <= stmin || stmax <= step) || KL.max_linesearch <= count + 1 || uinfo != 0)) ||
-                        (brackt && (stmax - stmin <= KL.xtol * stmax))) {
-                        step = xt;
-                    }
-#pragma unroll
-                    for (int q = 0; q < PPL; ++q)
-#pragma unroll
-                        for (int a = 0; a < D; ++a)
-                            x[q][a] = FAST ? fmaT((T)step, d[q][a], xp[q][a]) : xp[q][a] + (T)step * d[q][a];
-                    if constexpr (AXIS) x[0][2] = xp[0][2] + (T)step * (Q.interior[0] ? dz : T(0));
-                }
-
-                VIGO_TICK(t_pre);
-                if constexpr (AXIS) fx = eval_cost_grad_axis(KL, Q, grp, x, d, g, sums);
-                else fx = eval_cost_grad<T, GROUP, PPL, FAST, OBS, D>(KL, Q, x, d, g, sums);
-                VIGO_TICK(t_eval);
-                ++evals;
-                if (first) break;
-
-                const double dg = sums[4];
-                const double ftest1 = finit + step * dgtest;
-                ++count;
-
-                {
-                    int code = 0;
-                    if (fx <= ftest1 && fabs(dg) <= KL.gtol * (-dginit)) code = count;
-                    if (KL.max_linesearch <= count) code = LBERR_MAXIMUMLINESEARCH;
-                    if (brackt && (stmax - stmin) <= KL.xtol * stmax) code = LBERR_WIDTHTOOSMALL;
-                    if (step == stpmin && (ftest1 < fx || dgtest <= dg)) code = LBERR_MINIMUMSTEP;
-                    if (step == stpmax && fx <= ftest1 && dg <= dgtest) code = LBERR_MAXIMUMSTEP;
-                    if (brackt && ((step <= stmin || stmax <= step) || uinfo != 0)) code = LBERR_ROUNDING_ERROR;
-                    if (code != 0) { ls = code; break; }
-                }
-
-                const double cmin = KL.ftol <= KL.gtol ? KL.ftol : KL.gtol;
-                if (stage1 && fx <= ftest1 && cmin * dginit <= dg) stage1 = 0;
-
-                const bool mod = stage1 && ftest1 < fx && fx <= xf;
-                double axf = mod ? xf - xt * dgtest : xf, axd = mod ? xd - dgtest : xd;
-                double ayf = mod ? yf - yt * dgtest : yf, ayd = mod ? yd - dgtest : yd;
-                const double atf = mod ? fx - step * dgtest : fx, atd = mod ? dg - dgtest : dg;
-                VIGO_TICK(t_ls);
-                uinfo = trial_interval(xt, axf, axd, yt, ayf, ayd, step, atf, atd, stmin, stmax, brackt);
-                VIGO_TICK(t_trial);
-                xf = mod ? axf + xt * dgtest : axf;
-                yf = mod ? ayf + yt * dgtest : ayf;
-                xd = mod ? axd + dgtest : axd;
-                yd = mod ? ayd + dgtest : ayd;
-
-                if (brackt) {
-                    if (0.66 * prev_width <= fabs(yt - xt)) step = xt + 0.5 * (yt - xt);
-                    prev_width = width;
-                    width = fabs(yt - xt);
-                }
-            }
-        }
-
-        VIGO_TICK(t_ls);
-        double xnorm = sqrt(sums[5]), gnorm = sqrt(sums[6]);
-        if (first) {
-            first = false;
-#pragma unroll
-            for (int q = 0; q < PPL; ++q)
-#pragma unroll
-                for (int a = 0; a < D; ++a) d[q][a] = -g[q][a];
-            if constexpr (AXIS && VIGO_AXIS_CONV_FILTER) {
-                if (axis_converged(KL, sums[6], sums[5])) { ret = LB_ALREADY_MINIMIZED; break; }
-            } else {
-                if (xnorm < 1.0) xnorm = 1.0;
-                if (gnorm / xnorm <= KL.g_epsilon) { ret = LB_ALREADY_MINIMIZED; break; }
-            }
-            step = 1.0 / sqrt(sums[6]);
-            sums[4] = -sums[6];
-            k = 1;
-            end = 0;
-            continue;
-        }
-
-        if (ls < 0) {
-            if constexpr (AXIS) store_point_axis(A, b, Q, grp, Q.interior[0] ? x[0][0] : xp[0][0], Q.interior[0] ? x[0][2] : xp[0][2]);
-            else store_points<T, PPL>(A, b, Q, x);
-#pragma unroll
-            for (int q = 0; q < PPL; ++q)
-#pragma unroll
-                for (int a = 0; a < D; ++a) { x[q][a] = xp[q][a]; g[q][a] = gp[q][a]; }
-            if constexpr (AXIS) x[0][2] = xp[0][2];
-            ret = ls;
-            break;
-        }
-
-        if constexpr (AXIS && VIGO_AXIS_CONV_FILTER) {
-            if (axis_converged(KL, sums[6], sums[5])) { ret = LB_CONVERGENCE; break; }
-        } else {
-            if (xnorm < 1.0) xnorm = 1.0;
-            if (gnorm / xnorm <= KL.g_epsilon) { ret = LB_CONVERGENCE; break; }
-        }
-        if (KL.max_iterations != 0 && KL.max_iterations < k + 1) { ret = LBERR_MAXIMUMITERATION; break; }
-
-        T sv[PPL][3], yv[PPL][3];
-#pragma unroll
-        for (int q = 0; q < PPL; ++q) {
-#pragma unroll
-            for (int a = 0; a < D; ++a) { sv[q][a] = x[q][a] - xp[q][a]; yv[q][a] = g[q][a] - gp[q][a]; }
-            if (!REG1 && Q.interior[q]) {
-                HPair<T, D> hp;
-#pragma unroll
-                for (int a = 0; a < D; ++a) { hp.s[a] = sv[q][a]; hp.y[a] = yv[q][a]; }
-                hist_at(q, end) = hp;
-            }
-        }
-        double ysyy[2];
-        if constexpr (AXIS && VIGO_AXIS_PAIR_UPDATE) {
-            ys_yy_axis(yv[0][0], sv[0][0], ysyy[0], ysyy[1]);
-        } else {
-            ysyy[0] = dot_lane<FAST, T, PPL, D>(yv, sv);
-            ysyy[1] = dot_lane<FAST, T, PPL, D>(yv, yv);
-            if (D <= 2) ysyy[0] += 0.0;
-            group_sum<GROUP, 2>(ysyy);
-        }
-        const double ys = ysyy[0], yy = ysyy[1];
-        const YS ys_div = make_ys(ys, static_cast<YS*>(nullptr));
-        if (!REG1) ys_at(end) = ys_div;
-        const bool haveR = REG1 && k >= RH + 1;
-
-        const int bound = (m <= k) ? m : k;
-        const int newest = REG1 ? last : end;
-        if (!REG1) end = (end + 1 == m) ? 0 : end + 1;
-        ++k;
-#pragma unroll
-        for (int q = 0; q < PPL; ++q)
-#pragma unroll
-            for (int a = 0; a < D; ++a) d[q][a] = -g[q][a];
-
-        constexpr int kWin = 2;
-        T Ps[kWin][PPL][3], Py[kWin][PPL][3];
-        YS Pys[kWin];
-        auto fetch = [&](int age, T (&s_)[PPL][3], T (&y_)[PPL][3], YS& ys_) {
-            if (REG1 && age == 0) {
-#pragma unroll
-                for (int q = 0; q < PPL; ++q)
-#pragma unroll
-                    for (int a = 0; a < D; ++a) { s_[q][a] = sv[q][a]; y_[q][a] = yv[q][a]; }
-                ys_ = ys_div;
-                return;
-            }
-            if (REG1 && age >= 1 && age <= RH) {
-                const int j = (age - 1 < kRH && age >= 1) ? age - 1 : 0;
-#pragma unroll
-                for (int q = 0; q < PPL; ++q)
-#pragma unroll
-                    for (int a = 0; a < D; ++a) { s_[q][a] = sR[j][q][a]; y_[q][a] = yR[j][q][a]; }
-                ys_ = ysR[j];
-                return;
-            }
-            int slot = REG1 ? newest - (age - (RH + 1)) : newest - age;
-            if (slot < 0) slot += ms;
-#pragma unroll
-            for (int q = 0; q < PPL; ++q) {
-                const HPair<T, D> h = hist_at(q, slot);
-#pragma unroll
-                for (int a = 0; a < D; ++a) { s_[q][a] = h.s[a]; y_[q][a] = h.y[a]; }
-            }
-            ys_ = ys_at(slot);
-        };
-        auto two_loop = [&](auto steady_tag) -> bool {
-            constexpr bool STEADY = decltype(steady_tag)::value;
-            constexpr bool MARK = two_loop_mark<FAST>(decltype(steady_tag){});
-            double amin = 1.0, amax = 1.0;
-            const int bnd = STEADY ? kMaxMem : __builtin_amdgcn_readfirstlane(bound);
-            constexpr bool REGAL = STEADY || AXIS;
-            double al_reg[REGAL ? kMaxMem : 1];
-            constexpr int kRing = kMaxMem - (RH + 1);
-            constexpr int kFirstRing = RH + 1;
-            const int stepB = slotB;
-            const int lastU = STEADY ? __builtin_amdgcn_readfirstlane(last) : 0;
-            int curB = lastU * stepB;
-            auto ring_fetch = [&](T (&s_)[PPL][3], T (&y_)[PPL][3], YS& ys_) {
-#pragma unroll
-                for (int q = 0; q < PPL; ++q) {
-                    const HPair<T, D> h = *reinterpret_cast<const HPair<T, D>*>(reinterpret_cast<const char*>(hl[q]) + curB);
-#pragma unroll
-                    for (int a = 0; a < D; ++a) { s_[q][a] = h.s[a]; y_[q][a] = h.y[a]; }
-                }
-                ys_ = *reinterpret_cast<const YS*>(reinterpret_cast<const char*>(ys_l) + curB);
-            };
-            auto ring_older = [&]() {
-                curB -= stepB;
-                if (curB < 0) curB += kRing * stepB;
-            };
-            auto ring_newer = [&]() {
-                curB += stepB;
-                if (curB >= kRing * stepB) curB -= kRing * stepB;
-            };
-            auto ring_fetch_age = [&](int age, bool newer_next, T (&s_)[PPL][3], T (&y_)[PPL][3], YS& ys_) {
-                ring_fetch(s_, y_, ys_);
-                if (newer_next) ring_newer(); else ring_older();
-            };
-#pragma unroll
-            for (int q = 0; q < PPL; ++q)
-#pragma unroll
-                for (int a = 0; a < D; ++a) { Ps[0][q][a] = sv[q][a]; Py[0][q][a] = yv[q][a]; }
-            Pys[0] = ys_div;
-#pragma unroll
-            for (int age = 1; age < kWin; ++age)
-                if (age < bnd) {
-                    if (STEADY && age >= kFirstRing) ring_fetch_age(age, false, Ps[age], Py[age], Pys[age]);
-                    else fetch(age, Ps[age], Py[age], Pys[age]);
-                }
-#pragma unroll
-            for (int age = 0; age < kMaxMem; ++age) {
-                if (age < bnd) {
-                    const int w = age % kWin;
-                    double al = group_sum1<GROUP>(dot_lane<FAST, T, PPL, D>(Ps[w], d));
-                    al = over_ys<MARK>(al, Pys[w], amin, amax);
-                    if (REGAL) al_reg[REGAL ? age : 0] = al;
-                    else al_l[age * TPB] = al;
-                    {
-                        const T na = (T)(-al);
-#pragma unroll
-                        for (int q = 0; q < PPL; ++q)
-#pragma unroll
-                            for (int a = 0; a < D; ++a) d[q][a] = FAST ? fmaT(na, Py[w][q][a], d[q][a]) : d[q][a] + na * Py[w][q][a];
-                    }
-                    if (age + kWin < kMaxMem && age + kWin < bnd) {
-                        if (STEADY && age + kWin >= kFirstRing) ring_fetch_age(age + kWin, false, Ps[w], Py[w], Pys[w]);
-                        else fetch(age + kWin, Ps[w], Py[w], Pys[w]);
-                    }
-                }
-            }
-            if (STEADY) {
-#pragma unroll
-                for (int i = 0; i < kWin + 1; ++i) ring_newer();
-                asm volatile("" ::: "memory");
-            }
-            {
-                const T sc = (T)(ys / yy);
-#pragma unroll
-                for (int q = 0; q < PPL; ++q)
-#pragma unroll
-                    for (int a = 0; a < D; ++a) d[q][a] *= sc;
-            }
-#pragma unroll
-            for (int age = kMaxMem - 1; age >= 0; --age) {
-                if (age < bnd) {
-                    const int w = age % kWin;
-                    double beta = group_sum1<GROUP>(dot_lane<FAST, T, PPL, D>(Py[w], d));
-                    beta = over_ys<MARK>(beta, Pys[w], amin, amax);
-                    const double cod = (REGAL ? al_reg[REGAL ? age : 0] : al_l[age * TPB]) - beta;
-                    {
-                        const T co = (T)cod;
-#pragma unroll
-                        for (int q = 0; q < PPL; ++q)
-#pragma unroll
-                            for (int a = 0; a < D; ++a) d[q][a] = FAST ? fmaT(co, Ps[w][q][a], d[q][a]) : d[q][a] + co * Ps[w][q][a];
-                    }
-                    if (age - kWin >= 0) {
-                        if (STEADY && age - kWin >= kFirstRing) ring_fetch_age(age - kWin, true, Ps[w], Py[w], Pys[w]);
-                        else fetch(age - kWin, Ps[w], Py[w], Pys[w]);
-                    }
-                }
-            }
-            if (!MARK) return false;
-            bool bad = !(amin >= 0x1p-500) || !(amax <= 0x1p500);
-#pragma unroll
-            for (int q = 0; q < PPL; ++q)
-#pragma unroll
-                for (int a = 0; a < D; ++a) bad |= !(d[q][a] == d[q][a]);
-            return bad;
-        };
-        VIGO_TICK(t_upd);
-        if constexpr (AXIS) {
-            bool bad;
-            if (bound == kMaxMem && !__any(last != __builtin_amdgcn_readfirstlane(last))) bad = two_loop(TwoLoopTag<true, true>{});
-            else bad = two_loop(TwoLoopTag<false, true>{});
-            if (__any(bad)) {
-                asm volatile("" ::: "memory");
-                d[0][0] = -g[0][0];
-                two_loop(TwoLoopTag<false, false>{});
-            }
-        } else if (PPL == 1 && bound == kMaxMem && !__any(last != __builtin_amdgcn_readfirstlane(last))) {
-            if (__any(two_loop(std::true_type{}))) {
-                asm volatile("" ::: "memory");
-#pragma unroll
-                for (int q = 0; q < PPL; ++q)
-#pragma unroll
-                    for (int a = 0; a < D; ++a) d[q][a] = -g[q][a];
-                two_loop(std::false_type{});
-            }
-        } else {
-            two_loop(std::false_type{});
-        }
-        if constexpr (AXIS)
-            dz = __hiloint2double(__builtin_amdgcn_readfirstlane(__double2hiint(d[0][0])),
-                                  __builtin_amdgcn_readfirstlane(__double2loint(d[0][0])));
-#pragma unroll
-        for (int q = 0; q < PPL; ++q)
-#pragma unroll
-            for (int a = 0; a < D; ++a) d[q][a] = Q.interior[q] ? d[q][a] : T(0);
-        VIGO_TICK(t_two);
-        if (REG1) {
-            if (haveR && ms > 0) {
-#pragma unroll
-                for (int q = 0; q < PPL; ++q) {
-                    if (Q.interior[q]) {
-                        HPair<T, D> hp;
-#pragma unroll
-                        for (int a = 0; a < D; ++a) { hp.s[a] = sR[kRH - 1][q][a]; hp.y[a] = yR[kRH - 1][q][a]; }
-                        hist_at(q, end) = hp;
-                    }
-                }
-                ys_at(end) = ysR[kRH - 1];
-                last = end;
-                end = (end + 1 == ms) ? 0 : end + 1;
-            }
-#pragma unroll
-            for (int j = kRH - 1; j > 0; --j) {
-#pragma unroll
-                for (int q = 0; q < PPL; ++q)
-#pragma unroll
-                    for (int a = 0; a < D; ++a) { sR[j][q][a] = sR[j - 1][q][a]; yR[j][q][a] = yR[j - 1][q][a]; }
-                ysR[j] = ysR[j - 1];
-            }
-#pragma unroll
-            for (int q = 0; q < PPL; ++q)
-#pragma unroll
-                for (int a = 0; a < D; ++a) { sR[0][q][a] = sv[q][a]; yR[0][q][a] = yv[q][a]; }
-            ysR[0] = ys_div;
-        }
-        sums[4] = group_sum1<GROUP>(dot_lane<FAST, T, PPL, D>(g, d));
-        step = 1.0;
-        VIGO_TICK(t_tail);
-        VIGO_TICK(t_cal);
-    }
-
-    if (ret >= 0 || ret == LBERR_MAXIMUMITERATION) {
-        if constexpr (AXIS) store_point_axis(A, b, Q, grp, x[0][0], x[0][2]);
-        else store_points<T, PPL>(A, b, Q, x);
-    }
-#pragma unroll
-    for (int q = 0; q < PPL; ++q) {
-        if (Q.interior[q] && A.out_x) {
-            double* dst = A.out_x + ((size_t)b * NI + (Q.p0 + q - 3)) * 3;
-            if constexpr (AXIS) {
-                dst[grp] = (double)x[q][0];
-                if (grp == 0) dst[2] = (double)x[q][2];
-            } else {
-                dst[0] = (double)x[q][0]; dst[1] = (double)x[q][1]; dst[2] = (double)x[q][2];
-            }
-        }
-    }
-#if VIGO_PROFILE_SECTIONS
-    if (lane % GROUP == 0 && A.out_x) {
-        double* o = A.out_x + (size_t)b * NI * 3;
-        o[0] = t_eval; o[1] = t_ls; o[2] = t_upd; o[3] = t_two; o[4] = t_tail; o[5] = (double)k; o[6] = (double)evals;
-        o[7] = t_pre; o[8] = t_trial; o[9] = t_cal;
-    }
-#endif
-    if (lane % (kWave / TPB) == 0) {
-        if (A.out_status) A.out_status[(size_t)b * (A.status_stride ? A.status_stride : 1)] = ret;
-        if (A.out_fx) A.out_fx[b] = fx;
-        if (A.out_iters) A.out_iters[b] = k;
-        if (A.out_evals) A.out_evals[b] = evals;
+        if (grp) return;
+#if VIGO_FUSED_JOIN == 1
+        optimize_loaded<double, 32, 1, false, false, 3, true>(A, K, K, b, Q, x);
+#else
+#if VIGO_FUSED_JOIN == 0
+        SolveArgs A2 = A;
+#endif
+        LaneProblem<double, 1> Q2 = Q;
+        double x2[1][3] = {{x[0][0], x[0][1], x[0][2]}};
+#if VIGO_FUSED_JOIN == 2
+        optimize_solo((const void*)__builtin_amdgcn_kernarg_segment_ptr(), b, Q2, x2);
+#else
+        optimize_solo(A2, Kp, b, Q2, x2);
+#endif
+#endif
     }
 }
 
@@ -1554,6 +1052,14 @@
     return true;
 #endif
 }
+static inline bool fused_dispatch_on() {
+#if VIGO_EXP_AXIS_SWITCH
+    const char* e = getenv("VIGO_EXP_FUSE");
+    return !(e && e[0] == '0');
+#else
+    return true;
+#endif
+}
 
 int launch_optimize(hipStream_t s, const SolveArgs& a_in, const DevConst& k, const DevConst* kd, int precision, LaunchState& L) {
     static_assert(kOptimizeKeyCount <= 8 * (int)sizeof(L.lds_attr_set), "one bit per k_optimize instantiation");
@@ -1562,6 +1068,12 @@
                                             k.mem_size, L.simd_count, axis_dispatch_on());
     if (plan.count < 0) return (int)hipErrorInvalidValue;
     SolveArgs a = a_in;
+    if (const FusedLaunch f = fuse_optimize(plan, a_in.N, k.mem_size); f.fuse && fused_dispatch_on()) {
+        static_assert(solo_lds_bytes(32, kMaxMem) <= kLdsPerWorkgroup / 8, "two waves of the fused kernel per SIMD");
+        a.level_waves_elsewhere = 0;
+        hipLaunchKernelGGL(k_optimize_fused<2>, dim3(f.grid), dim3(kWave), f.lds, s, a, kd);
+        return (int)hipGetLastError();
+    }
     for (int i = 0; i < plan.count; ++i) {
         const PlannedLaunch& p = plan.launch[i];
         const SolveKernel kernel = kOptimizeKeys[p.key].obs ? optimize_kernel_with_obstacles(p.key) : optimize_kernel(p.key);
diff --git a/trajectory_planner_amd/csrc/vigo_solver_optimize.inc b/trajectory_planner_amd/csrc/vigo_solver_optimize.inc
--- /dev/null
+++ b/trajectory_planner_amd/csrc/vigo_solver_optimize.inc
@@ -0,0 +1,592 @@
+    static_assert(!MIXED || (D == 3 && OBS && PPL == 1), "mixed counts: the general kernel, one point per lane");
+    static_assert(PPL == 1 ? (RH >= 1 && RH <= 6) : RH == 0, "register-held history only with one point per lane");
+    constexpr bool AXIS = D == 1;
+    static_assert(!AXIS || (std::is_same<T, double>::value && GROUP == 32 && PPL == 1 && !FAST && !OBS),
+                  "the axis-per-lane layout: fp64 reference order, N <= 32, no obstacles");
+    static_assert(!SOLO || (D == 3 && GROUP == 32 && PPL == 1 && !OBS && !MIXED && kMaxMem <= GROUP),
+                  "one trajectory alone on half a wave: the general no-obstacle body of 32 x 1");
+#if VIGO_OPTIMIZE_ENTRY
+    const DevConst& K = *Kp;
+#endif
+    constexpr int TPB = (AXIS || SOLO) ? 1 : kWave / GROUP;
+    constexpr int COLS = SOLO ? 1 : kWave / GROUP;
+    extern __shared__ __align__(16) unsigned char lds_raw[];
+    const int N = A.N, NI = N - 6;
+    const int ROW = COLS * NI;
+    const int ROWP = ROW + 1;
+    using YS = YSv<FAST>;
+    constexpr int kYsSlotBytes = (TPB * (int)sizeof(YS) + 15) & ~15;
+    const int slotB = ROWP * (int)sizeof(HPair<T, D>) + kYsSlotBytes;
+    const int m = K.mem_size;
+#if VIGO_OPTIMIZE_ENTRY
+    const LoopConst<AXIS> KL(K);
+#endif
+    constexpr bool REG1 = (PPL == 1);
+    const int ms = REG1 ? (m > RH + 1 ? m - (RH + 1) : 0) : m;
+    HPair<T, D>* hist = reinterpret_cast<HPair<T, D>*>(lds_raw);
+    double* ys_tab = reinterpret_cast<double*>(lds_raw + (size_t)ms * slotB);
+
+    const int lane = threadIdx.x;
+    const int grp = lane / GROUP;
+    const int tg = AXIS ? 0 : grp;
+#if VIGO_OPTIMIZE_ENTRY
+    int b = blockIdx.x * TPB + tg;
+    if (A.active_idx) {
+        if (b >= *A.active_count) return;
+        b = A.active_idx[b];
+    } else if (b >= A.B) {
+        return;
+    }
+
+    LaneProblem<T, PPL> Q;
+    const bool valid_n = load_problem<T, GROUP, PPL, MIXED>(A, K, b, lane % GROUP, Q);
+    T x[PPL][3];
+    load_points<T, PPL>(A, b, Q, x);
+    set_level<T, GROUP, PPL>(K, Q, x);
+    if constexpr (AXIS) {
+        if (!Q.level) return;
+        x[0][0] = grp ? x[0][1] : x[0][0];
+        axis_guides(Q, grp);
+    } else {
+        const bool wave_level = __all(Q.level);
+        if (D == 2 && !wave_level) return;
+        if (D == 3 && A.level_waves_elsewhere && wave_level) return;
+    }
+#endif
+    const bool solved_elsewhere = D == 3 && !SOLO && A.level_waves_elsewhere == 2 && Q.level;
+#if VIGO_PROFILE_SECTIONS
+    long long tick_ = (long long)__builtin_readcyclecounter();
+    double t_eval = 0, t_ls = 0, t_upd = 0, t_two = 0, t_tail = 0, t_pre = 0, t_trial = 0, t_cal = 0;
+#endif
+    HPair<T, D>* hl[PPL];
+#pragma unroll
+    for (int q = 0; q < PPL; ++q) {
+        const int p = Q.p0 + q;
+        hl[q] = Q.interior[q] ? hist + (grp * NI + (p - 3)) : hist + ROW;
+    }
+    for (int slot = lane; slot < ms; slot += kWave) {
+        HPair<T, D> zero;
+#pragma unroll
+        for (int a = 0; a < D; ++a) zero.s[a] = zero.y[a] = T(0);
+        *reinterpret_cast<HPair<T, D>*>(lds_raw + (size_t)slot * slotB + (size_t)ROW * sizeof(HPair<T, D>)) = zero;
+    }
+    __syncthreads();
+    if (solved_elsewhere) return;
+    if (MIXED && !valid_n) {
+        if (lane % GROUP == 0 && A.out_status) A.out_status[(size_t)b * (A.status_stride ? A.status_stride : 1)] = LBERR_INVALID_N;
+        return;
+    }
+    YS* ys_l = reinterpret_cast<YS*>(lds_raw + (size_t)ROWP * sizeof(HPair<T, D>)) + tg;
+    double* al_l = ys_tab + tg;
+    auto hist_at = [&](int q, int slot) -> HPair<T, D>& {
+        return *reinterpret_cast<HPair<T, D>*>(reinterpret_cast<char*>(hl[q]) + (size_t)slot * slotB);
+    };
+    auto ys_at = [&](int slot) -> YS& { return *reinterpret_cast<YS*>(reinterpret_cast<char*>(ys_l) + (size_t)slot * slotB); };
+    if (!OBS) { Q.obs = nullptr; Q.o_begin = Q.o_end = 0; }
+    if (OBS && A.obs) {
+        constexpr int kEnt = kObsTabEntries<GROUP>;
+        double* tab = ys_tab + (size_t)m * TPB + (size_t)grp * kObsTabDoubles<GROUP>;
+        const int cnt = Q.o_end - Q.o_begin;
+        const int steps = K.pred_num / 2 + 1;
+        int fit = kEnt / steps;
+        if (fit > kObsTabObs) fit = kObsTabObs;
+        Q.o_tab = cnt < fit ? cnt : fit;
+        Q.o_steps = steps;
+        Q.obs_tab = tab;
+        Q.obs_size = tab + 3 * kEnt;
+        for (int e = lane % GROUP; e < Q.o_tab * steps; e += GROUP) {
+            const int j = e / steps, n = 2 * (e - j * steps);
+            const double* o = A.obs + 9 * (size_t)(Q.o_begin + j);
+            const T tn = (T)((double)n * K.ts);
+            tab[3 * e + 0] = (double)((T)o[0] + tn * (T)o[3]);
+            tab[3 * e + 1] = (double)((T)o[1] + tn * (T)o[4]);
+            tab[3 * e + 2] = (double)((T(1) - (T)(n / K.pred_num) * T(0.2)) * (T)K.thr_dyn);
+        }
+        for (int j = lane % GROUP; j < Q.o_tab; j += GROUP) {
+            const double* o = A.obs + 9 * (size_t)(Q.o_begin + j);
+            const T hx = (T)o[6] / 2, hy = (T)o[7] / 2;
+            tab[3 * kEnt + j] = (double)(T)sqrt(hx * hx + hy * hy);
+        }
+        __syncthreads();
+    }
+
+    T g[PPL][3], xp[PPL][3], gp[PPL][3], d[PPL][3];
+#pragma unroll
+    for (int q = 0; q < PPL; ++q)
+#pragma unroll
+        for (int a = 0; a < 3; ++a) g[q][a] = xp[q][a] = gp[q][a] = d[q][a] = T(0);
+    constexpr int kRH = RH > 0 ? RH : 1;
+    T sR[kRH][PPL][3], yR[kRH][PPL][3];
+    YS ysR[kRH]{};
+#pragma unroll
+    for (int q = 0; q < PPL; ++q)
+#pragma unroll
+        for (int a = 0; a < 3; ++a)
+#pragma unroll
+            for (int j = 0; j < kRH; ++j) sR[j][q][a] = yR[j][q][a] = T(0);
+    T dz = T(-0.0);
+    double sums[7];
+    int evals = 0;
+    int ret = LBERR_UNKNOWN;
+    int k = 0, end = 0, last = 0;
+    double fx = 0.0, step = 0.0;
+    bool first = true;
+
+    for (;;) {
+        int ls = 0;
+        if constexpr (AXIS && (VIGO_AXIS_LS_FIRST_TESTS || VIGO_AXIS_LS_FIRST_SETUP)) {
+            constexpr bool kTests = VIGO_AXIS_LS_FIRST_TESTS, kDefer = VIGO_AXIS_LS_FIRST_SETUP == 1;
+            const LsParams P{KL.min_step, KL.max_step, KL.ftol, KL.gtol, KL.xtol, KL.max_linesearch};
+            LsState S;
+            fresh_reg(S.dginit); fresh_reg(S.finit); fresh_reg(S.dgtest); fresh_reg(S.width); fresh_reg(S.prev_width);
+            fresh_reg(S.xt); fresh_reg(S.xf); fresh_reg(S.xd); fresh_reg(S.yt); fresh_reg(S.yf); fresh_reg(S.yd);
+            fresh_reg(S.stmin); fresh_reg(S.stmax);
+            fresh_reg(S.count); fresh_reg(S.brackt); fresh_reg(S.stage1); fresh_reg(S.uinfo);
+            double step0 = step;
+            auto move_x = [&]() {
+                x[0][0] = xp[0][0] + step * d[0][0];
+                x[0][2] = xp[0][2] + step * (Q.interior[0] ? dz : 0.0);
+            };
+            bool run = true;
+            if (!first) {
+                xp[0][0] = x[0][0]; gp[0][0] = g[0][0];
+                xp[0][2] = x[0][2];
+                ls = kDefer ? ls_first_begin(P, S, step, fx, sums[4]) : ls_begin(P, S, step, fx, sums[4]);
+                run = ls == 0;
+                if (run) {
+                    if constexpr (kDefer) ls_first_setup(P, step);
+                    else ls_setup(P, S, step);
+                    move_x();
+                }
+            }
+            while (run) {
+                VIGO_TICK(t_pre);
+                fx = eval_cost_grad_axis(KL, Q, grp, x, d, g, sums);
+                VIGO_TICK(t_eval);
+                ++evals;
+                if (first) break;
+
+                const double dg = sums[4];
+                const double ftest1 = ls_ftest1(S, step);
+                ++S.count;
+                if ((kTests || kDefer) && S.count == 1) {
+                    if constexpr (kTests) {
+                        const int code = ls_first_exit_code(P, S, step, fx, dg, ftest1);
+                        if (__any(code != 0)) { ls = code; break; }
+                    }
+                    if constexpr (kDefer) {
+                        hold_in_reg(step0);
+                        ls_first_reject(P, S, step0);
+                        hold_in_reg(S.xt); hold_in_reg(S.xf); hold_in_reg(S.xd); hold_in_reg(S.yt); hold_in_reg(S.yf); hold_in_reg(S.yd);
+                        hold_in_reg(S.width); hold_in_reg(S.prev_width); hold_in_reg(S.stmin); hold_in_reg(S.stmax);
+                        hold_in_reg(S.brackt); hold_in_reg(S.stage1); hold_in_reg(S.uinfo);
+                    }
+                }
+                if (!kTests || S.count != 1) {
+                    const int code = ls_exit_code(P, S, step, fx, dg, ftest1);
+                    if (code != 0) { ls = code; break; }
+                }
+                VIGO_TICK(t_ls);
+                ls_update(P, S, step, fx, dg, ftest1);
+                VIGO_TICK(t_trial);
+                ls_setup(P, S, step);
+                move_x();
+            }
+        } else {
+            int count = 0, brackt = 0, stage1 = 1, uinfo = 0;
+            double dginit = 0.0, finit = 0.0, dgtest = 0.0, width = 0.0, prev_width = 0.0;
+            double xt = 0., xf = 0., xd = 0., yt = 0., yf = 0., yd = 0.;
+            const double stpmin = KL.min_step, stpmax = KL.max_step;
+            bool run = true;
+            if (!first) {
+#pragma unroll
+                for (int q = 0; q < PPL; ++q)
+#pragma unroll
+                    for (int a = 0; a < D; ++a) { xp[q][a] = x[q][a]; gp[q][a] = g[q][a]; }
+                if constexpr (AXIS) xp[0][2] = x[0][2];
+                dginit = sums[4];
+                if (step <= 0.) { ls = LBERR_INVALIDPARAMETERS; run = false; }
+                else if (0 < dginit) { ls = LBERR_INCREASEGRADIENT; run = false; }
+                finit = fx;
+                dgtest = KL.ftol * dginit;
+                width = stpmax - stpmin;
+                prev_width = 2.0 * width;
+                xt = yt = 0.;
+                xf = yf = finit;
+                xd = yd = dginit;
+            }
+            while (run) {
+                double stmin = 0., stmax = 0.;
+                if (!first) {
+                    if (brackt) {
+                        stmin = xt <= yt ? xt : yt;
+                        stmax = xt >= yt ? xt : yt;
+                    } else {
+                        stmin = xt;
+                        stmax = step + 4.0 * (step - xt);
+                    }
+                    if (step < stpmin) step = stpmin;
+                    if (stpmax < step) step = stpmax;
+                    if ((brackt && ((step <= stmin || stmax <= step) || KL.max_linesearch <= count + 1 || uinfo != 0)) ||
+                        (brackt && (stmax - stmin <= KL.xtol * stmax))) {
+                        step = xt;
+                    }
+#pragma unroll
+                    for (int q = 0; q < PPL; ++q)
+#pragma unroll
+                        for (int a = 0; a < D; ++a)
+                            x[q][a] = FAST ? fmaT((T)step, d[q][a], xp[q][a]) : xp[q][a] + (T)step * d[q][a];
+                    if constexpr (AXIS) x[0][2] = xp[0][2] + (T)step * (Q.interior[0] ? dz : T(0));
+                }
+
+                VIGO_TICK(t_pre);
+                if constexpr (AXIS) fx = eval_cost_grad_axis(KL, Q, grp, x, d, g, sums);
+                else fx = eval_cost_grad<T, GROUP, PPL, FAST, OBS, D>(KL, Q, x, d, g, sums);
+                VIGO_TICK(t_eval);
+                ++evals;
+                if (first) break;
+
+                const double dg = sums[4];
+                const double ftest1 = finit + step * dgtest;
+                ++count;
+
+                {
+                    int code = 0;
+                    if (fx <= ftest1 && fabs(dg) <= KL.gtol * (-dginit)) code = count;
+                    if (KL.max_linesearch <= count) code = LBERR_MAXIMUMLINESEARCH;
+                    if (brackt && (stmax - stmin) <= KL.xtol * stmax) code = LBERR_WIDTHTOOSMALL;
+                    if (step == stpmin && (ftest1 < fx || dgtest <= dg)) code = LBERR_MINIMUMSTEP;
+                    if (step == stpmax && fx <= ftest1 && dg <= dgtest) code = LBERR_MAXIMUMSTEP;
+                    if (brackt && ((step <= stmin || stmax <= step) || uinfo != 0)) code = LBERR_ROUNDING_ERROR;
+                    if (code != 0) { ls = code; break; }
+                }
+
+                const double cmin = KL.ftol <= KL.gtol ? KL.ftol : KL.gtol;
+                if (stage1 && fx <= ftest1 && cmin * dginit <= dg) stage1 = 0;
+
+                const bool mod = stage1 && ftest1 < fx && fx <= xf;
+                double axf = mod ? xf - xt * dgtest : xf, axd = mod ? xd - dgtest : xd;
+                double ayf = mod ? yf - yt * dgtest : yf, ayd = mod ? yd - dgtest : yd;
+                const double atf = mod ? fx - step * dgtest : fx, atd = mod ? dg - dgtest : dg;
+                VIGO_TICK(t_ls);
+                uinfo = trial_interval(xt, axf, axd, yt, ayf, ayd, step, atf, atd, stmin, stmax, brackt);
+                VIGO_TICK(t_trial);
+                xf = mod ? axf + xt * dgtest : axf;
+                yf = mod ? ayf + yt * dgtest : ayf;
+                xd = mod ? axd + dgtest : axd;
+                yd = mod ? ayd + dgtest : ayd;
+
+                if (brackt) {
+                    if (0.66 * prev_width <= fabs(yt - xt)) step = xt + 0.5 * (yt - xt);
+                    prev_width = width;
+                    width = fabs(yt - xt);
+                }
+            }
+        }
+
+        VIGO_TICK(t_ls);
+        double xnorm = sqrt(sums[5]), gnorm = sqrt(sums[6]);
+        if (first) {
+            first = false;
+#pragma unroll
+            for (int q = 0; q < PPL; ++q)
+#pragma unroll
+                for (int a = 0; a < D; ++a) d[q][a] = -g[q][a];
+            if constexpr (AXIS && VIGO_AXIS_CONV_FILTER) {
+                if (axis_converged(KL, sums[6], sums[5])) { ret = LB_ALREADY_MINIMIZED; break; }
+            } else {
+                if (xnorm < 1.0) xnorm = 1.0;
+                if (gnorm / xnorm <= KL.g_epsilon) { ret = LB_ALREADY_MINIMIZED; break; }
+            }
+            step = 1.0 / sqrt(sums[6]);
+            sums[4] = -sums[6];
+            k = 1;
+            end = 0;
+            continue;
+        }
+
+        if (ls < 0) {
+            if constexpr (AXIS) store_point_axis(A, b, Q, grp, Q.interior[0] ? x[0][0] : xp[0][0], Q.interior[0] ? x[0][2] : xp[0][2]);
+            else store_points<T, PPL>(A, b, Q, x);
+#pragma unroll
+            for (int q = 0; q < PPL; ++q)
+#pragma unroll
+                for (int a = 0; a < D; ++a) { x[q][a] = xp[q][a]; g[q][a] = gp[q][a]; }
+            if constexpr (AXIS) x[0][2] = xp[0][2];
+            ret = ls;
+            break;
+        }
+
+        if constexpr (AXIS && VIGO_AXIS_CONV_FILTER) {
+            if (axis_converged(KL, sums[6], sums[5])) { ret = LB_CONVERGENCE; break; }
+        } else {
+            if (xnorm < 1.0) xnorm = 1.0;
+            if (gnorm / xnorm <= KL.g_epsilon) { ret = LB_CONVERGENCE; break; }
+        }
+        if (KL.max_iterations != 0 && KL.max_iterations < k + 1) { ret = LBERR_MAXIMUMITERATION; break; }
+
+        T sv[PPL][3], yv[PPL][3];
+#pragma unroll
+        for (int q = 0; q < PPL; ++q) {
+#pragma unroll
+            for (int a = 0; a < D; ++a) { sv[q][a] = x[q][a] - xp[q][a]; yv[q][a] = g[q][a] - gp[q][a]; }
+            if (!REG1 && Q.interior[q]) {
+                HPair<T, D> hp;
+#pragma unroll
+                for (int a = 0; a < D; ++a) { hp.s[a] = sv[q][a]; hp.y[a] = yv[q][a]; }
+                hist_at(q, end) = hp;
+            }
+        }
+        double ysyy[2];
+        if constexpr (AXIS && VIGO_AXIS_PAIR_UPDATE) {
+            ys_yy_axis(yv[0][0], sv[0][0], ysyy[0], ysyy[1]);
+        } else {
+            ysyy[0] = dot_lane<FAST, T, PPL, D>(yv, sv);
+            ysyy[1] = dot_lane<FAST, T, PPL, D>(yv, yv);
+            if (D <= 2) ysyy[0] += 0.0;
+            group_sum<GROUP, 2>(ysyy);
+        }
+        const double ys = ysyy[0], yy = ysyy[1];
+        const YS ys_div = make_ys(ys, static_cast<YS*>(nullptr));
+        if (!REG1) ys_at(end) = ys_div;
+        const bool haveR = REG1 && k >= RH + 1;
+
+        const int bound = (m <= k) ? m : k;
+        const int newest = REG1 ? last : end;
+        if (!REG1) end = (end + 1 == m) ? 0 : end + 1;
+        ++k;
+#pragma unroll
+        for (int q = 0; q < PPL; ++q)
+#pragma unroll
+            for (int a = 0; a < D; ++a) d[q][a] = -g[q][a];
+
+        constexpr int kWin = 2;
+        T Ps[kWin][PPL][3], Py[kWin][PPL][3];
+        YS Pys[kWin];
+        auto fetch = [&](int age, T (&s_)[PPL][3], T (&y_)[PPL][3], YS& ys_) {
+            if (REG1 && age == 0) {
+#pragma unroll
+                for (int q = 0; q < PPL; ++q)
+#pragma unroll
+                    for (int a = 0; a < D; ++a) { s_[q][a] = sv[q][a]; y_[q][a] = yv[q][a]; }
+                ys_ = ys_div;
+                return;
+            }
+            if (REG1 && age >= 1 && age <= RH) {
+                const int j = (age - 1 < kRH && age >= 1) ? age - 1 : 0;
+#pragma unroll
+                for (int q = 0; q < PPL; ++q)
+#pragma unroll
+                    for (int a = 0; a < D; ++a) { s_[q][a] = sR[j][q][a]; y_[q][a] = yR[j][q][a]; }
+                ys_ = ysR[j];
+                return;
+            }
+            int slot = REG1 ? newest - (age - (RH + 1)) : newest - age;
+            if (slot < 0) slot += ms;
+#pragma unroll
+            for (int q = 0; q < PPL; ++q) {
+                const HPair<T, D> h = hist_at(q, slot);
+#pragma unroll
+                for (int a = 0; a < D; ++a) { s_[q][a] = h.s[a]; y_[q][a] = h.y[a]; }
+            }
+            ys_ = ys_at(slot);
+        };
+        auto two_loop = [&](auto steady_tag) -> bool {
+            constexpr bool STEADY = decltype(steady_tag)::value;
+            constexpr bool MARK = two_loop_mark<FAST>(decltype(steady_tag){});
+            double amin = 1.0, amax = 1.0;
+            const int bnd = STEADY ? kMaxMem : __builtin_amdgcn_readfirstlane(bound);
+            constexpr bool REGAL = STEADY || AXIS;
+            double al_reg[REGAL ? kMaxMem : 1];
+            constexpr int kRing = kMaxMem - (RH + 1);
+            constexpr int kFirstRing = RH + 1;
+            const int stepB = slotB;
+            const int lastU = STEADY ? __builtin_amdgcn_readfirstlane(last) : 0;
+            int curB = lastU * stepB;
+            auto ring_fetch = [&](T (&s_)[PPL][3], T (&y_)[PPL][3], YS& ys_) {
+#pragma unroll
+                for (int q = 0; q < PPL; ++q) {
+                    const HPair<T, D> h = *reinterpret_cast<const HPair<T, D>*>(reinterpret_cast<const char*>(hl[q]) + curB);
+#pragma unroll
+                    for (int a = 0; a < D; ++a) { s_[q][a] = h.s[a]; y_[q][a] = h.y[a]; }
+                }
+                ys_ = *reinterpret_cast<const YS*>(reinterpret_cast<const char*>(ys_l) + curB);
+            };
+            auto ring_older = [&]() {
+                curB -= stepB;
+                if (curB < 0) curB += kRing * stepB;
+            };
+            auto ring_newer = [&]() {
+                curB += stepB;
+                if (curB >= kRing * stepB) curB -= kRing * stepB;
+            };
+            auto ring_fetch_age = [&](int age, bool newer_next, T (&s_)[PPL][3], T (&y_)[PPL][3], YS& ys_) {
+                ring_fetch(s_, y_, ys_);
+                if (newer_next) ring_newer(); else ring_older();
+            };
+#pragma unroll
+            for (int q = 0; q < PPL; ++q)
+#pragma unroll
+                for (int a = 0; a < D; ++a) { Ps[0][q][a] = sv[q][a]; Py[0][q][a] = yv[q][a]; }
+            Pys[0] = ys_div;
+#pragma unroll
+            for (int age = 1; age < kWin; ++age)
+                if (age < bnd) {
+                    if (STEADY && age >= kFirstRing) ring_fetch_age(age, false, Ps[age], Py[age], Pys[age]);
+                    else fetch(age, Ps[age], Py[age], Pys[age]);
+                }
+#pragma unroll
+            for (int age = 0; age < kMaxMem; ++age) {
+                if (age < bnd) {
+                    const int w = age % kWin;
+                    double al = group_sum1<GROUP>(dot_lane<FAST, T, PPL, D>(Ps[w], d));
+                    al = over_ys<MARK>(al, Pys[w], amin, amax);
+                    if (REGAL) al_reg[REGAL ? age : 0] = al;
+                    else al_l[age * TPB] = al;
+                    {
+                        const T na = (T)(-al);
+#pragma unroll
+                        for (int q = 0; q < PPL; ++q)
+#pragma unroll
+                            for (int a = 0; a < D; ++a) d[q][a] = FAST ? fmaT(na, Py[w][q][a], d[q][a]) : d[q][a] + na * Py[w][q][a];
+                    }
+                    if (age + kWin < kMaxMem && age + kWin < bnd) {
+                        if (STEADY && age + kWin >= kFirstRing) ring_fetch_age(age + kWin, false, Ps[w], Py[w], Pys[w]);
+                        else fetch(age + kWin, Ps[w], Py[w], Pys[w]);
+                    }
+                }
+            }
+            if (STEADY) {
+#pragma unroll
+                for (int i = 0; i < kWin + 1; ++i) ring_newer();
+                asm volatile("" ::: "memory");
+            }
+            {
+                const T sc = (T)(ys / yy);
+#pragma unroll
+                for (int q = 0; q < PPL; ++q)
+#pragma unroll
+                    for (int a = 0; a < D; ++a) d[q][a] *= sc;
+            }
+#pragma unroll
+            for (int age = kMaxMem - 1; age >= 0; --age) {
+                if (age < bnd) {
+                    const int w = age % kWin;
+                    double beta = group_sum1<GROUP>(dot_lane<FAST, T, PPL, D>(Py[w], d));
+                    beta = over_ys<MARK>(beta, Pys[w], amin, amax);
+                    const double cod = (REGAL ? al_reg[REGAL ? age : 0] : al_l[age * TPB]) - beta;
+                    {
+                        const T co = (T)cod;
+#pragma unroll
+                        for (int q = 0; q < PPL; ++q)
+#pragma unroll
+                            for (int a = 0; a < D; ++a) d[q][a] = FAST ? fmaT(co, Ps[w][q][a], d[q][a]) : d[q][a] + co * Ps[w][q][a];
+                    }
+                    if (age - kWin >= 0) {
+                        if (STEADY && age - kWin >= kFirstRing) ring_fetch_age(age - kWin, true, Ps[w], Py[w], Pys[w]);
+                        else fetch(age - kWin, Ps[w], Py[w], Pys[w]);
+                    }
+                }
+            }
+            if (!MARK) return false;
+            bool bad = !(amin >= 0x1p-500) || !(amax <= 0x1p500);
+#pragma unroll
+            for (int q = 0; q < PPL; ++q)
+#pragma unroll
+                for (int a = 0; a < D; ++a) bad |= !(d[q][a] == d[q][a]);
+            return bad;
+        };
+        VIGO_TICK(t_upd);
+        if constexpr (AXIS) {
+            bool bad;
+            if (bound == kMaxMem && !__any(last != __builtin_amdgcn_readfirstlane(last))) bad = two_loop(TwoLoopTag<true, true>{});
+            else bad = two_loop(TwoLoopTag<false, true>{});
+            if (__any(bad)) {
+                asm volatile("" ::: "memory");
+                d[0][0] = -g[0][0];
+                two_loop(TwoLoopTag<false, false>{});
+            }
+        } else if (PPL == 1 && bound == kMaxMem && !__any(last != __builtin_amdgcn_readfirstlane(last))) {
+            if (__any(two_loop(std::true_type{}))) {
+                asm volatile("" ::: "memory");
+#pragma unroll
+                for (int q = 0; q < PPL; ++q)
+#pragma unroll
+                    for (int a = 0; a < D; ++a) d[q][a] = -g[q][a];
+                two_loop(std::false_type{});
+            }
+        } else {
+            two_loop(std::false_type{});
+        }
+        if constexpr (AXIS)
+            dz = __hiloint2double(__builtin_amdgcn_readfirstlane(__double2hiint(d[0][0])),
+                                  __builtin_amdgcn_readfirstlane(__double2loint(d[0][0])));
+#pragma unroll
+        for (int q = 0; q < PPL; ++q)
+#pragma unroll
+            for (int a = 0; a < D; ++a) d[q][a] = Q.interior[q] ? d[q][a] : T(0);
+        VIGO_TICK(t_two);
+        if (REG1) {
+            if (haveR && ms > 0) {
+#pragma unroll
+                for (int q = 0; q < PPL; ++q) {
+                    if (Q.interior[q]) {
+                        HPair<T, D> hp;
+#pragma unroll
+                        for (int a = 0; a < D; ++a) { hp.s[a] = sR[kRH - 1][q][a]; hp.y[a] = yR[kRH - 1][q][a]; }
+                        hist_at(q, end) = hp;
+                    }
+                }
+                ys_at(end) = ysR[kRH - 1];
+                last = end;
+                end = (end + 1 == ms) ? 0 : end + 1;
+            }
+#pragma unroll
+            for (int j = kRH - 1; j > 0; --j) {
+#pragma unroll
+                for (int q = 0; q < PPL; ++q)
+#pragma unroll
+                    for (int a = 0; a < D; ++a) { sR[j][q][a] = sR[j - 1][q][a]; yR[j][q][a] = yR[j - 1][q][a]; }
+                ysR[j] = ysR[j - 1];
+            }
+#pragma unroll
+            for (int q = 0; q < PPL; ++q)
+#pragma unroll
+                for (int a = 0; a < D; ++a) { sR[0][q][a] = sv[q][a]; yR[0][q][a] = yv[q][a]; }
+            ysR[0] = ys_div;
+        }
+        sums[4] = group_sum1<GROUP>(dot_lane<FAST, T, PPL, D>(g, d));
+        step = 1.0;
+        VIGO_TICK(t_tail);
+        VIGO_TICK(t_cal);
+    }
+
+    if (ret >= 0 || ret == LBERR_MAXIMUMITERATION) {
+        if constexpr (AXIS) store_point_axis(A, b, Q, grp, x[0][0], x[0][2]);
+        else store_points<T, PPL>(A, b, Q, x);
+    }
+#pragma unroll
+    for (int q = 0; q < PPL; ++q) {
+        if (Q.interior[q] && A.out_x) {
+            double* dst = A.out_x + ((size_t)b * NI + (Q.p0 + q - 3)) * 3;
+            if constexpr (AXIS) {
+                dst[grp] = (double)x[q][0];
+                if (grp == 0) dst[2] = (double)x[q][2];
+            } else {
+                dst[0] = (double)x[q][0]; dst[1] = (double)x[q][1]; dst[2] = (double)x[q][2];
+            }
+        }
+    }
+#if VIGO_PROFILE_SECTIONS
+    if (lane % GROUP == 0 && A.out_x) {
+        double* o = A.out_x + (size_t)b * NI * 3;
+        o[0] = t_eval; o[1] = t_ls; o[2] = t_upd; o[3] = t_two; o[4] = t_tail; o[5] = (double)k; o[6] = (double)evals;
+        o[7] = t_pre; o[8] = t_trial; o[9] = t_cal;
+    }
+#endif
+    if (lane % (kWave / TPB) == 0) {
+        if (A.out_status) A.out_status[(size_t)b * (A.status_stride ? A.status_stride : 1)] = ret;
+        if (A.out_fx) A.out_fx[b] = fx;
+        if (A.out_iters) A.out_iters[b] = k;
+        if (A.out_evals) A.out_evals[b] = evals;
+    }
diff --git a/trajectory_planner_amd/csrc/vigo_solver_plan.hpp b/trajectory_planner_amd/csrc/vigo_solver_plan.hpp
--- a/trajectory_planner_amd/csrc/vigo_solver_plan.hpp
+++ b/trajectory_planner_amd/csrc/vigo_solver_plan.hpp
@@ -103,6 +103,17 @@
     return p;
 }
 
+constexpr size_t solo_lds_bytes(int N, int m) {
+    const int ms = m > 2 ? m - 2 : 0;
+    return (size_t)ms * (((size_t)(N - 6) + 1) * hpair_bytes(8, 3) + ysv_bytes(false)) + (size_t)m * sizeof(double);
+}
+struct FusedLaunch { bool fuse; int grid; size_t lds; };
+inline FusedLaunch fuse_optimize(const OptimizePlan& p, int N, int mem_size) {
+    if (p.count != 2 || kOptimizeKeys[p.launch[0].key].d != 1) return FusedLaunch{false, 0, 0};
+    const size_t axis = p.launch[0].lds, solo = solo_lds_bytes(N, mem_size);
+    return FusedLaunch{true, p.launch[0].grid, axis > solo ? axis : solo};
+}
+
 constexpr int kMixedMaxStride = 64;
 constexpr OptimizeKey kOptimizeMixedKeys[] = {
     {kF32, 32, 1, 2, true, 3, 1}, {kF32, 32, 1, 1, true, 3, 1}, {kF32, 64, 1, 2, true, 3, 1}, {kF32, 64, 1, 1, true, 3, 1},
```
